# KleistLab/ADAPTed

Measured on NVIDIA B200. Metric: reads_per_sec, higher is better.
Workload: dtype f64 traces / f32 statistics / fp16-split tensor-core convolutions / i16 input

## Files before the change

adapted_b200/csrc/adb_cnn.cuh:

```cuda
#pragma once
#include "adb_series_median.cuh"
#include <cuda_fp16.h>
#include <float.h>

#include "adb_common.cuh"
#include "adb_ctx.cuh"
#include "adb_select.cuh"
#include <algorithm>

#define ADB_CNN_NPARAMS 58882
#define CNN_C 64
#define CNN_K 7
#define CNN_SCORE_EXCL (-5.0f)
#define CNN_W1 0
#define CNN_B1 (CNN_W1 + 64 * 7)
#define CNN_W2 (CNN_B1 + 64)
#define CNN_B2 (CNN_W2 + 64 * 64 * 7)
#define CNN_W3 (CNN_B2 + 64)
#define CNN_B3 (CNN_W3 + 64 * 64 * 7)
#define CNN_W4 (CNN_B3 + 64)
#define CNN_B4 (CNN_W4 + 64 * 2 * 7)

#define CNN_TILE 96
#define CNN_TILE_IN 104
#define CNN_THREADS 192

struct SmemKeys {
    const float *p;
    __device__ __forceinline__ uint32_t operator()(int j) const { return f32_key(p[j]); }
};
struct SmemDevKeys {
    const float *p;
    float med;
    __device__ __forceinline__ uint32_t operator()(int j) const { return f32_key(fabsf(__fsub_rn(p[j], med))); }
};
struct KeyF32Id {
    __device__ __forceinline__ float operator()(uint32_t k) const { return key_f32(k); }
};

template <class F>
__device__ __forceinline__ float cnn_block_mean(F f, int factor) {
    return __fdiv_rn(np_sum_f32_leaf(f, factor), (float)factor);
}

__global__ void __launch_bounds__(256) cnn_prep_kernel(BatchDev B, int A0, int f, int L, float *x) {
    extern __shared__ __align__(16) unsigned char smem[];
    float *ds = (float *)smem;
    unsigned char *scr = smem + (((size_t)L * 4 + 15) & ~(size_t)15);
    SelScratch S = sel_scratch_from(scr);
    uint32_t *kbuf = (uint32_t *)(scr + ((ADB_SEL_SMEM_BYTES + 15) & ~15));
    const int r = blockIdx.x;
    const ReadSrc src = make_src(B, r);
    int nv;
    {
        const int span = B.m - A0;
        if (span <= 0) nv = 0;
        else if (src.n >= B.m) nv = L;
        else nv = (src.n > A0) ? (src.n - A0) / f : 0;
        nv = min(nv, L);
    }
    for (int b = threadIdx.x; b < nv; b += blockDim.x) {
        const int j0 = A0 + b * f;
        ds[b] = cnn_block_mean([&](int k) { const int j = j0 + k; return (j < B.m) ? src.pa(j) : 0.0f; }, f);
    }
    __syncthreads();
    float med = CUDART_NAN_F, mad = CUDART_NAN_F;
    if (nv > 0) {
        uint32_t kmin, kmax;
        SmemKeys K{ds};
        cta_key_minmax(K, nv, kmin, kmax, S);
        med = cta_median_keys(K, KeyF32Id(), nv, kmin, kmax, S, kbuf);
        SmemDevKeys D{ds, med};
        const float dmax = fmaxf(fabsf(__fsub_rn(key_f32(kmax), med)), fabsf(__fsub_rn(key_f32(kmin), med)));
        mad = cta_median_keys(D, KeyF32Id(), nv, f32_key(0.0f), f32_key(dmax), S, kbuf);
    }
    float *xr = x + (size_t)r * L;
    for (int b = threadIdx.x; b < L; b += blockDim.x) {
        float v = CNN_SCORE_EXCL;
        if (b < nv) {
            v = __fdiv_rn(__fsub_rn(ds[b], med), mad);
            if (!(v == v)) v = CNN_SCORE_EXCL;
            else if (v == CUDART_INF_F) v = FLT_MAX;
            else if (v == -CUDART_INF_F) v = -FLT_MAX;
        }
        xr[b] = v;
    }
}

#define PREP_WARPS 4
#define PREP_CHUNK_BINS 320
__host__ __device__ inline size_t cnn_prep_warp_smem(int L) { return (size_t)PREP_WARPS * (2 * ((L + 3) & ~3) + SM_NCAND + 4) * 4; }
__global__ void __launch_bounds__(PREP_WARPS * 32) cnn_prep_warp_kernel(BatchDev B, int A0, int f, int L, float *x) {
    extern __shared__ __align__(16) unsigned char smem[];
    const int warp = threadIdx.x >> 5, lane = threadIdx.x & 31;
    const int Lp = (L + 3) & ~3;
    float *ds = (float *)smem + (size_t)warp * (2 * Lp + SM_NCAND + 4);
    uint32_t *keys = (uint32_t *)(ds + Lp), *cand = keys + Lp;
    __shared__ uint64_t pbar[PREP_WARPS];
    if (threadIdx.x < PREP_WARPS) mbar_init(&pbar[threadIdx.x], 1);
    __syncthreads();
    uint32_t pphase = 0;
    for (int r = blockIdx.x * PREP_WARPS + warp; r < B.n_reads; r += gridDim.x * PREP_WARPS) {
        const ReadSrc src = make_src(B, r);
        int nv;
        {
            const int span = B.m - A0;
            if (span <= 0) nv = 0;
            else if (src.n >= B.m) nv = L;
            else nv = (src.n > A0) ? (src.n - A0) / f : 0;
            nv = min(nv, L);
        }
        const int nvp = (nv + 3) & ~3;
        if (lane == 0) {
            const int rn = r + gridDim.x * PREP_WARPS;
            if (rn < B.n_reads) {
                const ReadSrc nx = make_src(B, rn);
                if (nx.i16 != nullptr && nx.n > A0 + 16) {
                    const uintptr_t p0 = ((uintptr_t)(nx.i16 + A0) + 15) & ~(uintptr_t)15;
                    const uint32_t nbytes = (uint32_t)(((uintptr_t)(nx.i16 + min(nx.n, B.m)) - p0) & ~(uintptr_t)15);
                    if (nbytes) asm volatile("cp.async.bulk.prefetch.L2.global [%0], %1;" ::"l"(p0), "r"(nbytes) : "memory");
                }
            }
        }
        uint32_t mn = 0xffffffffu, mx = 0u;
        {
            int16_t *raw = reinterpret_cast<int16_t *>(keys);
            const int16_t *g0 = src.i16 + A0;
            const int cbins = min(PREP_CHUNK_BINS, (Lp * 4 - 16) / (2 * f));
            const int n_have = min(src.n, B.m) - A0;
            for (int b0 = 0; b0 < nv; b0 += cbins) {
                const int nbin = min(cbins, nv - b0), ns = min(nbin * f, n_have - b0 * f);
                const int16_t *gs = g0 + (size_t)b0 * f;
                const int shift = (int)(((uintptr_t)gs & 15) >> 1);
                const int head = min((8 - shift) & 7, ns);
                const int body = (ns - head) & ~7;
                asm volatile("fence.proxy.async.shared::cta;" ::: "memory");
                __syncwarp();
                if (lane == 0 && body > 0) {
                    mbar_expect_tx(&pbar[warp], (uint32_t)body * 2);
                    tma_bulk_g2s(raw + shift + head, gs + head, (uint32_t)body * 2, &pbar[warp]);
                }
                for (int i = lane; i < head; i += 32) raw[shift + i] = gs[i];
                for (int i = head + body + lane; i < ns; i += 32) raw[shift + i] = gs[i];
                if (body > 0) { mbar_wait(&pbar[warp], pphase); pphase ^= 1; }
                __syncwarp();
                const int16_t *rs = raw + shift;
                for (int b = lane; b < nbin; b += 32) {
                    const int16_t *p = rs + b * f;
                    const int left = ns - b * f;
                    const float v = cnn_block_mean([&](int k) { return (k < left) ? __fmul_rn(__fadd_rn((float)(int)p[k], src.coff), src.cscale) : 0.0f; }, f);
                    ds[b0 + b] = v;
                    const uint32_t k0 = f32_key(v);
                    mn = min(mn, k0); mx = max(mx, k0);
                }
                __syncwarp();
            }
            for (int b = lane; b < nv; b += 32) keys[b] = f32_key(ds[b]);
        }
        if (lane < nvp - nv) keys[nv + lane] = 0xffffffffu;
        mn = __reduce_min_sync(ADB_FULL, mn);
        mx = __reduce_max_sync(ADB_FULL, mx);
        __syncwarp();
        float med = CUDART_NAN_F, mad = CUDART_NAN_F;
        if (nv > 0) {
            const SmKeys K{reinterpret_cast<const uint4 *>(keys), nullptr};
            const unsigned rank = (unsigned)(nv - 1) >> 1;
            uint32_t a, b2;
            bool hb;
            warp_select2(K, nvp >> 2, 0u, false, nvp, rank, mn, mx, cand, a, b2, hb);
            med = (nv & 1) ? key_f32(a) : __fdiv_rn(__fadd_rn(key_f32(a), key_f32(b2)), 2.0f);
            __syncwarp();
            mn = 0xffffffffu; mx = 0u;
            for (int b = lane; b < nv; b += 32) {
                const uint32_t k = f32_key(fabsf(__fsub_rn(ds[b], med)));
                keys[b] = k;
                mn = min(mn, k); mx = max(mx, k);
            }
            mn = __reduce_min_sync(ADB_FULL, mn);
            mx = __reduce_max_sync(ADB_FULL, mx);
            __syncwarp();
            warp_select2(K, nvp >> 2, 0u, false, nvp, rank, mn, mx, cand, a, b2, hb);
            mad = (nv & 1) ? key_f32(a) : __fdiv_rn(__fadd_rn(key_f32(a), key_f32(b2)), 2.0f);
        }
        float *xr = x + (size_t)r * L;
        for (int b = lane; b < L; b += 32) {
            float v = CNN_SCORE_EXCL;
            if (b < nv) {
                v = __fdiv_rn(__fsub_rn(ds[b], med), mad);
                if (!(v == v)) v = CNN_SCORE_EXCL;
                else if (v == CUDART_INF_F) v = FLT_MAX;
                else if (v == -CUDART_INF_F) v = -FLT_MAX;
            }
            xr[b] = v;
        }
        __syncwarp();
    }
}

__global__ void cnn_pack_weights_kernel(const float *w, float *packed ) {
    const int i = blockIdx.x * blockDim.x + threadIdx.x;
    if (i >= 2 * CNN_C * CNN_K * CNN_C) return;
    const int layer = i / (CNN_C * CNN_K * CNN_C);
    const int rem = i % (CNN_C * CNN_K * CNN_C);
    const int ci = rem / (CNN_K * CNN_C), k = (rem / CNN_C) % CNN_K, co = rem % CNN_C;
    const float *src = w + (layer == 0 ? CNN_W2 : CNN_W3);
    packed[i] = src[(co * CNN_C + ci) * CNN_K + k];
}

template <bool FUSE_L1>
__global__ void __launch_bounds__(CNN_THREADS, 1) cnn_conv64_kernel(const float *in, float *out, const float *packed_w,
                                                                   const float *bias, const float *w1, const float *b1,
                                                                   int n_reads, int Lx, int L1, int LP, const int *only) {
    if (only) {
        if (only[-1] == 0) return;
        const int tiles_per_read = (L1 + CNN_TILE - 1) / CNN_TILE, n_tiles = n_reads * tiles_per_read;
        bool mine = false;
        for (int tile = blockIdx.x; tile < n_tiles && !mine; tile += gridDim.x) mine = only[tile / tiles_per_read] != 0;
        if (!__syncthreads_or(mine)) return;
    }
    extern __shared__ __align__(16) float sm[];
    float *Ws = sm;
    float *Is = Ws + CNN_C * CNN_K * CNN_C;
    float *Xs = Is + CNN_C * CNN_TILE_IN;
    float *W1s = Xs + 3 * (CNN_TILE + 6) + 8;
    for (int i = threadIdx.x; i < CNN_C * CNN_K * CNN_C; i += blockDim.x) Ws[i] = packed_w[i];
    if (FUSE_L1) {
        for (int i = threadIdx.x; i < CNN_C * CNN_K; i += blockDim.x) W1s[i] = w1[i];
        for (int i = threadIdx.x; i < CNN_C; i += blockDim.x) W1s[CNN_C * CNN_K + i] = b1[i];
    }
    __syncthreads();
    const int tiles_per_read = (L1 + CNN_TILE - 1) / CNN_TILE;
    const int n_tiles = n_reads * tiles_per_read;
    const int cg = threadIdx.x / 24, tg = threadIdx.x % 24;
    const int co0 = cg * 8, tp = tg * 4;
    float bv[8];
#pragma unroll
    for (int c = 0; c < 8; c++) bv[c] = bias[co0 + c];
    for (int tile = blockIdx.x; tile < n_tiles; tile += gridDim.x) {
        const int r = tile / tiles_per_read, t0 = (tile % tiles_per_read) * CNN_TILE;
        if (only && !only[r]) continue;
        __syncthreads();
        if (FUSE_L1) {
            const float *xr = in + (size_t)r * Lx;
            const int x0 = 3 * (t0 - 3) - 3, nx = 3 * (CNN_TILE + 6) + 6;
            for (int i = threadIdx.x; i < nx; i += blockDim.x) {
                const int j = x0 + i;
                Xs[i] = (j >= 0 && j < Lx) ? xr[j] : 0.0f;
            }
            __syncthreads();
            for (int i = threadIdx.x; i < CNN_C * (CNN_TILE + 6); i += blockDim.x) {
                const int ci = i / (CNN_TILE + 6), q = i % (CNN_TILE + 6);
                const int p = t0 - 3 + q;
                float v = 0.0f;
                if (p >= 0 && p < L1) {
                    float a = W1s[CNN_C * CNN_K + ci];
#pragma unroll
                    for (int k = 0; k < CNN_K; k++) a = fmaf(W1s[ci * CNN_K + k], Xs[3 * q + k], a);
                    v = fmaxf(a, 0.0f);
                }
                Is[ci * CNN_TILE_IN + q] = v;
            }
        } else {
            const float *ar = in + (size_t)r * CNN_C * LP;
            for (int i = threadIdx.x; i < CNN_C * (CNN_TILE + 6); i += blockDim.x) {
                const int ci = i / (CNN_TILE + 6), q = i % (CNN_TILE + 6);
                const int p = t0 - 3 + q;
                Is[ci * CNN_TILE_IN + q] = (p >= 0 && p < L1) ? ar[(size_t)ci * LP + p] : 0.0f;
            }
        }
        __syncthreads();
        float acc[8][4];
#pragma unroll
        for (int c = 0; c < 8; c++)
#pragma unroll
            for (int t = 0; t < 4; t++) acc[c][t] = bv[c];
#pragma unroll 2
        for (int ci = 0; ci < CNN_C; ci++) {
            float iv[10];
            const float *ip = Is + ci * CNN_TILE_IN + tp;
#pragma unroll
            for (int q = 0; q < 10; q++) iv[q] = ip[q];
            const float *wp = Ws + ci * CNN_K * CNN_C + co0;
#pragma unroll
            for (int k = 0; k < CNN_K; k++) {
                const float4 wa = *(const float4 *)(wp + k * CNN_C);
                const float4 wb = *(const float4 *)(wp + k * CNN_C + 4);
                const float wv[8] = {wa.x, wa.y, wa.z, wa.w, wb.x, wb.y, wb.z, wb.w};
#pragma unroll
                for (int c = 0; c < 8; c++)
#pragma unroll
                    for (int t = 0; t < 4; t++) acc[c][t] = fmaf(wv[c], iv[t + k], acc[c][t]);
            }
        }
        float *orow = out + (size_t)r * CNN_C * LP;
        const int p0 = t0 + tp;
        if (p0 < L1) {
#pragma unroll
            for (int c = 0; c < 8; c++) {
                float4 v = make_float4(fmaxf(acc[c][0], 0.f), fmaxf(acc[c][1], 0.f), fmaxf(acc[c][2], 0.f), fmaxf(acc[c][3], 0.f));
                float *dst = orow + (size_t)(co0 + c) * LP + p0;
                if (p0 + 3 < LP) *(float4 *)dst = v;
                else {
                    if (p0 < LP) dst[0] = v.x;
                    if (p0 + 1 < LP) dst[1] = v.y;
                    if (p0 + 2 < LP) dst[2] = v.z;
                }
            }
        }
    }
}

__host__ __device__ inline size_t cnn_conv_smem_bytes() {
    return (size_t)(CNN_C * CNN_K * CNN_C + CNN_C * CNN_TILE_IN + 3 * (CNN_TILE + 6) + 8 + CNN_C * CNN_K + CNN_C) * 4;
}

#define CNN_CONVT_THREADS 192
__global__ void __launch_bounds__(CNN_CONVT_THREADS) cnn_convT_kernel(const float *act, const float *w4, const float *b4, int L1, int LP,
                                                        int Lout, float *scores, const int *only) {
    if (only && (only[-1] == 0 || only[blockIdx.y] == 0)) return;
    __shared__ __align__(16) float ws[CNN_C * 16];
    for (int i = threadIdx.x; i < CNN_C * 16; i += blockDim.x) {
        const int ci = i >> 4, e = i & 15, co = e >> 3, k = e & 7;
        ws[i] = (k < CNN_K) ? w4[(ci * 2 + co) * CNN_K + k] : 0.0f;
    }
    __syncthreads();
    const int r = blockIdx.y;
    const int u = blockIdx.x * blockDim.x + threadIdx.x;
    if (3 * u >= Lout) return;
    const float *ar = act + (size_t)r * CNN_C * LP;
    const float bias0 = b4[0], bias1 = b4[1];
    float o[2][3] = {{bias0, bias0, bias0}, {bias1, bias1, bias1}};
    const bool has_m = (u - 1 >= 0) && (u - 1 < L1), has_c = u < L1, has_p = u + 1 < L1;
#pragma unroll 8
    for (int ci = 0; ci < CNN_C; ci++) {
        const float *ap = ar + (size_t)ci * LP;
        const float xm = has_m ? ap[u - 1] : 0.0f, xc = has_c ? ap[u] : 0.0f, xp = has_p ? ap[u + 1] : 0.0f;
        const float4 wa = *reinterpret_cast<const float4 *>(ws + ci * 16), wb = *reinterpret_cast<const float4 *>(ws + ci * 16 + 4);
        const float4 wc = *reinterpret_cast<const float4 *>(ws + ci * 16 + 8), wd = *reinterpret_cast<const float4 *>(ws + ci * 16 + 12);
        if (has_p) { o[0][0] = fmaf(xp, wa.x, o[0][0]); o[1][0] = fmaf(xp, wc.x, o[1][0]); }
        if (has_c) { o[0][0] = fmaf(xc, wa.w, o[0][0]); o[1][0] = fmaf(xc, wc.w, o[1][0]); }
        if (has_m) { o[0][0] = fmaf(xm, wb.z, o[0][0]); o[1][0] = fmaf(xm, wd.z, o[1][0]); }
        if (has_p) { o[0][1] = fmaf(xp, wa.y, o[0][1]); o[1][1] = fmaf(xp, wc.y, o[1][1]); }
        if (has_c) { o[0][1] = fmaf(xc, wb.x, o[0][1]); o[1][1] = fmaf(xc, wd.x, o[1][1]); }
        if (has_p) { o[0][2] = fmaf(xp, wa.z, o[0][2]); o[1][2] = fmaf(xp, wc.z, o[1][2]); }
        if (has_c) { o[0][2] = fmaf(xc, wb.y, o[0][2]); o[1][2] = fmaf(xc, wd.y, o[1][2]); }
    }
#pragma unroll
    for (int c = 0; c < 3; c++) {
        const int j = 3 * u + c;
        if (j < Lout) {
            scores[((size_t)r * 2 + 0) * Lout + j] = o[0][c];
            scores[((size_t)r * 2 + 1) * Lout + j] = o[1][c];
        }
    }
}

__device__ __forceinline__ bool np_better(float v, int i, float bv, int bi) {
    const bool vn = !(v == v), bn = !(bv == bv);
    if (vn != bn) return vn;
    if (vn) return i < bi;
    return v > bv || (v == bv && i < bi);
}

__device__ int cta_argmax(const float *p, int n, float *sv, int *si) {
    float bv = -CUDART_INF_F;
    int bi = 0x7fffffff;
    for (int i = threadIdx.x; i < n; i += blockDim.x) {
        const float v = p[i];
        if (bi == 0x7fffffff || np_better(v, i, bv, bi)) { bv = v; bi = i; }
    }
#pragma unroll
    for (int o = 16; o > 0; o >>= 1) {
        const float ov = __shfl_xor_sync(ADB_FULL, bv, o);
        const int oi = __shfl_xor_sync(ADB_FULL, bi, o);
        if (oi != 0x7fffffff && (bi == 0x7fffffff || np_better(ov, oi, bv, bi))) { bv = ov; bi = oi; }
    }
    __syncthreads();
    if ((threadIdx.x & 31) == 0) { sv[threadIdx.x >> 5] = bv; si[threadIdx.x >> 5] = bi; }
    __syncthreads();
    bv = sv[0]; bi = si[0];
    for (int w = 1; w < (int)(blockDim.x >> 5); w++)
        if (si[w] != 0x7fffffff && (bi == 0x7fffffff || np_better(sv[w], si[w], bv, bi))) { bv = sv[w]; bi = si[w]; }
    __syncthreads();
    return bi == 0x7fffffff ? 0 : bi;
}

__global__ void __launch_bounds__(256) cnn_mask_kernel(float *scores, int Lout, int n_adapter_bins, int k, int *apos,
                                                       int *ppos) {
    __shared__ float sv[8];
    __shared__ int si[8];
    const int r = blockIdx.x;
    float *c0 = scores + ((size_t)r * 2) * Lout, *c1 = c0 + Lout;
    const int a = cta_argmax(c0, min(n_adapter_bins, Lout), sv, si);
    int p = 0;
    if (k >= 1) {
        for (int j = threadIdx.x; j < a; j += blockDim.x) c1[j] = CNN_SCORE_EXCL;
        __syncthreads();
        p = cta_argmax(c1, Lout, sv, si);
        if (k > 1)
            for (int j = p + 1 + threadIdx.x; j < Lout; j += blockDim.x) c1[j] = CNN_SCORE_EXCL;
    }
    if (threadIdx.x == 0) { apos[r] = a; ppos[r] = p; }
}

struct FlatView {
    const float *scores;
    int Lout;
    int r0, nr;
    __device__ __forceinline__ float at(long long g) const {
        const int rr = (int)(g / Lout), j = (int)(g % Lout);
        return scores[((size_t)(r0 + rr) * 2 + 1) * Lout + j];
    }
    __device__ __forceinline__ long long size() const { return (long long)nr * Lout; }
};

#define CNN_PK_CAP 832

__global__ void __launch_bounds__(128) cnn_peaks_kernel(const float *scores, int Lout, int batch_size, int n_reads,
                                                        long long *pk_pos, int *pk_cnt) {
    __shared__ int wcount[4];
    __shared__ int base_sh;
    const int r = blockIdx.x;
    const int mb = r / batch_size;
    FlatView V{scores, Lout, mb * batch_size, min(batch_size, n_reads - mb * batch_size)};
    const long long N = V.size();
    const long long g0 = (long long)(r - V.r0) * Lout;
    const float *rowp = scores + ((size_t)r * 2 + 1) * Lout;
    if (threadIdx.x == 0) base_sh = 0;
    __syncthreads();
    for (int jb = 0; jb < Lout; jb += blockDim.x) {
        const int j = jb + threadIdx.x;
        long long mid = -1;
        if (j < Lout) {
            const long long i = g0 + j;
            if (i >= 1 && i < N - 1) {
                auto val = [&](long long g) { const long long jj = g - g0; return (jj >= 0 && jj < Lout) ? rowp[jj] : V.at(g); };
                const float xi = rowp[j];
                if (val(i - 1) < xi) {
                    long long ia = i + 1;
                    while (ia < N - 1 && val(ia) == xi) ia++;
                    if (val(ia) < xi) mid = (i + ia - 1) / 2;
                }
            }
        }
        const unsigned m = __ballot_sync(ADB_FULL, mid >= 0);
        if ((threadIdx.x & 31) == 0) wcount[threadIdx.x >> 5] = __popc(m);
        __syncthreads();
        int off = base_sh;
        for (int w = 0; w < (int)(threadIdx.x >> 5); w++) off += wcount[w];
        if (mid >= 0) {
            const int pos = off + __popc(m & ((1u << (threadIdx.x & 31)) - 1u));
            if (pos < CNN_PK_CAP) pk_pos[(size_t)r * CNN_PK_CAP + pos] = mid;
        }
        __syncthreads();
        if (threadIdx.x == 0) base_sh += wcount[0] + wcount[1] + wcount[2] + wcount[3];
        __syncthreads();
    }
    if (threadIdx.x == 0) pk_cnt[r] = min(base_sh, CNN_PK_CAP);
}

#define CNN_WS_CAP 2560
#define CNN_WS_SORT 4096
__global__ void __launch_bounds__(128) cnn_topk_kernel(const float *scores, int Lout, int batch_size, int n_reads, int k,
                                                       int dist, const long long *pk_pos, const int *pk_cnt, int *cand,
                                                       int *ncand) {
    __shared__ long long pos[CNN_WS_CAP];
    __shared__ float hgt[CNN_WS_CAP];
    __shared__ unsigned short ord[CNN_WS_CAP];
    __shared__ unsigned char keep[CNN_WS_CAP];
    __shared__ int n_sh;
    const int r = blockIdx.x;
    const int mb = r / batch_size;
    FlatView V{scores, Lout, mb * batch_size, min(batch_size, n_reads - mb * batch_size)};
    const int rl = r - V.r0;
    __shared__ int take_sh[2];
    const int c_mid = pk_cnt[r];
    const long long lo = (long long)rl * Lout, hi = lo + Lout;
    if (threadIdx.x == 0) {
        int tl = 0, tr = 0;
        const long long *pm = pk_pos + (size_t)r * CNN_PK_CAP;
        long long first_pos = (c_mid > 0) ? pm[0] : 0x7fffffffffffffffLL, last_pos = (c_mid > 0) ? pm[c_mid - 1] : -1;
        if (rl > 0) {
            const long long *pl = pk_pos + (size_t)(r - 1) * CNN_PK_CAP;
            const int cl = pk_cnt[r - 1];
            long long nxt = first_pos;
            while (tl < cl) {
                const long long p = pl[cl - 1 - tl];
                if (!(p >= lo || (dist > 0 && nxt != 0x7fffffffffffffffLL && nxt - p < dist))) break;
                nxt = p; tl++;
                if (last_pos < 0) last_pos = p;
            }
        }
        if (rl + 1 < V.nr && dist > 0 && last_pos >= 0) {
            const long long *pr = pk_pos + (size_t)(r + 1) * CNN_PK_CAP;
            const int cr = pk_cnt[r + 1];
            long long prv = last_pos;
            while (tr < cr && pr[tr] - prv < dist) { prv = pr[tr]; tr++; }
        }
        take_sh[0] = tl; take_sh[1] = tr;
    }
    __syncthreads();
    int n = 0;
    for (int part = 0; part < 3; part++) {
        const int rr = r - 1 + part;
        int c, first;
        if (part == 0) { c = take_sh[0]; first = (c > 0) ? pk_cnt[r - 1] - c : 0; }
        else if (part == 1) { c = c_mid; first = 0; }
        else { c = take_sh[1]; first = 0; }
        for (int i = threadIdx.x; i < c; i += blockDim.x) {
            if (n + i < CNN_WS_CAP) {
                const long long p = pk_pos[(size_t)rr * CNN_PK_CAP + first + i];
                pos[n + i] = p;
                hgt[n + i] = V.at(p);
                keep[n + i] = 2;
            }
        }
        n = min(n + c, CNN_WS_CAP);
    }
    auto over = [&](int t, int i) { const float ht = hgt[t], hi_ = hgt[i]; return (ht > hi_) || (ht == hi_ && t > i); };
    __syncthreads();
    if (dist > 0) {
        bool pending = true;
        while (__syncthreads_or(pending)) {
            pending = false;
            unsigned char newst[(CNN_WS_CAP + 127) / 128];
            int cnt = 0;
            for (int i = threadIdx.x; i < n; i += blockDim.x, cnt++) {
                unsigned char st = keep[i];
                if (st == 2) {
                    bool killed = false, wait = false;
                    for (int t = i - 1; t >= 0 && pos[i] - pos[t] < dist; t--)
                        if (over(t, i)) { const unsigned char s2 = keep[t]; killed |= (s2 == 1); wait |= (s2 == 2); }
                    for (int t = i + 1; t < n && pos[t] - pos[i] < dist; t++)
                        if (over(t, i)) { const unsigned char s2 = keep[t]; killed |= (s2 == 1); wait |= (s2 == 2); }
                    if (killed) st = 0;
                    else if (!wait) st = 1;
                    else pending = true;
                }
                newst[cnt] = st;
            }
            __syncthreads();
            cnt = 0;
            for (int i = threadIdx.x; i < n; i += blockDim.x, cnt++) keep[i] = newst[cnt];
        }
    } else {
        for (int i = threadIdx.x; i < n; i += blockDim.x) keep[i] = 1;
    }
    __syncthreads();
    if (threadIdx.x == 0) n_sh = 0;
    __syncthreads();
    for (int i = threadIdx.x; i < n; i += blockDim.x)
        if (keep[i] == 1 && pos[i] >= lo && pos[i] < hi) ord[atomicAdd(&n_sh, 1)] = (unsigned short)i;
    __syncthreads();
    const int ns = n_sh;
    for (int a = threadIdx.x; a < ns; a += blockDim.x) {
        const int i = ord[a];
        const float h = hgt[i];
        int rank = 0;
        for (int b = 0; b < ns; b++) {
            const int j = ord[b];
            const float hj = hgt[j];
            rank += (hj > h) || (hj == h && j < i);
        }
        if (rank < k) cand[(size_t)r * k + rank] = (int)(pos[i] - lo);
    }
    if (threadIdx.x == 0) ncand[r] = ns;
}

__global__ void __launch_bounds__(256) cnn_shift_kernel(const int *apos, const int *ppos, const int *cand, const int *ncand,
                                                        int batch_size, int n_reads, int k, int ds, int A0, int *given) {
    __shared__ int wtot[8];
    __shared__ int carry;
    const int mb = blockIdx.x;
    const int r0 = mb * batch_size, nr = min(batch_size, n_reads - r0);
    const int stride = 1 + max(k, 1);
    if (threadIdx.x == 0) carry = 0;
    for (int i = threadIdx.x; i < nr; i += blockDim.x) {
        int *g = given + (size_t)(r0 + i) * stride;
        const int a = apos[r0 + i];
        g[0] = (a == 0) ? 0 : a * ds + A0;
        for (int t = 0; t < max(k, 1); t++) g[1 + t] = 0;
        if (k == 1) { const int p = ppos[r0 + i]; g[1] = (p == 0) ? 0 : p * ds + A0; }
    }
    __syncthreads();
    if (k <= 1) return;
    for (int base = 0; base < nr; base += blockDim.x) {
        const int i = base + threadIdx.x;
        const int has = (i < nr && ncand[r0 + i] > 0) ? 1 : 0;
        const unsigned m = __ballot_sync(ADB_FULL, has);
        if ((threadIdx.x & 31) == 0) wtot[threadIdx.x >> 5] = __popc(m);
        __syncthreads();
        int off = carry;
        for (int w = 0; w < (int)(threadIdx.x >> 5); w++) off += wtot[w];
        if (has) {
            const int row = off + __popc(m & ((1u << (threadIdx.x & 31)) - 1u));
            int *g = given + (size_t)(r0 + row) * stride;
            const int nc = min(ncand[r0 + i], k);
            for (int t = 0; t < nc; t++) {
                const int p = cand[(size_t)(r0 + i) * k + t];
                g[1 + t] = (p == 0) ? 0 : p * ds + A0;
            }
        }
        __syncthreads();
        if (threadIdx.x == 0) { int s = 0; for (int w = 0; w < 8; w++) s += wtot[w]; carry += s; }
        __syncthreads();
    }
}

struct CnnDims {
    int Lx, L1, LP, Lout;
};
static CnnDims cnn_dims(int m, int A0, int f) {
    CnnDims d;
    d.Lx = (std::max(m - A0, 0) + f - 1) / f;
    d.L1 = (d.Lx + 2 * 3 - CNN_K) / 3 + 1;
    d.LP = (d.L1 + 3) & ~3;
    d.Lout = (d.L1 - 1) * 3 - 2 * 3 + CNN_K;
    return d;
}

__global__ void cnn_tc_pack_weights_kernel(const float *w, __half *packed);
static int cnn_tc_launch_setup();
#define ADB_CT_SLOTS 4
#define ADB_CT_FLOATS (2 * 64 * 8 + 64)
__constant__ float adb_c_convT[ADB_CT_SLOTS][ADB_CT_FLOATS];

__global__ void cnn_ct_pack_kernel(const float *w4 , const float *b3, float *out) {
    const int i = blockIdx.x * blockDim.x + threadIdx.x;
    if (i < 1024) {
        const int co = i >> 9, ci = (i >> 3) & 63, k = i & 7;
        out[i] = (k < CNN_K) ? w4[(ci * 2 + co) * CNN_K + k] : 0.0f;
    } else if (i < ADB_CT_FLOATS) {
        out[i] = b3[i - 1024];
    }
}

static void cnn_tc_launch(int layer, const void *in, void *out, const __half *wp, const float *bias, const float *w1,
                          const float *b1, int n_reads, int Lx, int L1, int LP, int *redo, int sm_count, cudaStream_t st, int cslot = -1);
static size_t cnn_tc_a0t_bytes_per_read(int L1);
static int cnn_tc_a0t_rows_host(int L1);

static int cnn_forward_dev(adb_ctx *ctx, const float *x, int n, const CnnDims &D, const float *w_dev, float *scores,
                           cudaStream_t st) {
    if (ctx->cnn_w.ensure(sizeof(float) * 2 * CNN_C * CNN_K * CNN_C)) { set_err("cudaMalloc cnn weights"); return ADB_ERR_CUDA; }
    float *packed = (float *)ctx->cnn_w.p;
    {
        KernelTimer t(ctx, 6, st);
        cnn_pack_weights_kernel<<<(2 * CNN_C * CNN_K * CNN_C + 255) / 256, 256, 0, st>>>(w_dev, packed);
    }
    ctx->launches += 1;
    const size_t act_per_read = (size_t)CNN_C * D.LP * sizeof(float);
    const int chunk = (int)std::max<size_t>(1, std::min<size_t>((size_t)n, ((size_t)1 << 30) / act_per_read));
    if (ctx->cnn_act0.ensure(act_per_read * chunk) || ctx->cnn_act1.ensure(act_per_read * chunk)) {
        set_err("cudaMalloc cnn activations");
        return ADB_ERR_CUDA;
    }
    const size_t smem = cnn_conv_smem_bytes();
    CUDA_TRY(cudaFuncSetAttribute(cnn_conv64_kernel<true>, cudaFuncAttributeMaxDynamicSharedMemorySize, (int)smem));
    CUDA_TRY(cudaFuncSetAttribute(cnn_conv64_kernel<false>, cudaFuncAttributeMaxDynamicSharedMemorySize, (int)smem));
    float *a0 = (float *)ctx->cnn_act0.p, *a1 = (float *)ctx->cnn_act1.p;
    const bool use_tc = !ctx->opt_cnn_fp32;
    __half *wtc = nullptr;
    unsigned char *a0t = nullptr;
    int *redo = nullptr;
    int cslot = -1;
    if (use_tc) {
        const size_t wbytes = sizeof(__half) * 2 * CNN_K * 2 * 4096;
        if (ctx->cnn_wtc.ensure(wbytes + sizeof(int) * ((size_t)chunk + 4))) { set_err("cudaMalloc cnn tc weights"); return ADB_ERR_CUDA; }
        wtc = (__half *)ctx->cnn_wtc.p;
        redo = (int *)((unsigned char *)ctx->cnn_wtc.p + wbytes) + 4;
        {
            KernelTimer t(ctx, 6, st);
            cnn_tc_pack_weights_kernel<<<(2 * CNN_K * 4096 + 255) / 256, 256, 0, st>>>(w_dev, wtc);
        }
        ctx->launches += 1;
        if (ctx->ct_slot >= 0 && !getenv("ADB_NO_CONST_CONVT")) {
            if (ctx->cnn_ct.ensure(sizeof(float) * ADB_CT_FLOATS)) { set_err("cudaMalloc cnn constants"); return ADB_ERR_CUDA; }
            cnn_ct_pack_kernel<<<(ADB_CT_FLOATS + 255) / 256, 256, 0, st>>>(w_dev + CNN_W4, w_dev + CNN_B3, (float *)ctx->cnn_ct.p);
            CUDA_TRY(cudaMemcpyToSymbolAsync(adb_c_convT, ctx->cnn_ct.p, sizeof(float) * ADB_CT_FLOATS,
                                             sizeof(float) * ADB_CT_FLOATS * (size_t)ctx->ct_slot, cudaMemcpyDeviceToDevice, st));
            ctx->launches += 1;
            cslot = ctx->ct_slot;
        }
        if (cnn_tc_launch_setup()) { set_err("cudaFuncSetAttribute cnn tc"); return ADB_ERR_CUDA; }
        const size_t a0t_bytes = cnn_tc_a0t_bytes_per_read(D.L1) * (size_t)chunk;
        const void *before = ctx->cnn_a0t.p;
        const size_t cap_before = ctx->cnn_a0t.cap;
        if (ctx->cnn_a0t.ensure(a0t_bytes)) { set_err("cudaMalloc cnn a0t"); return ADB_ERR_CUDA; }
        if (ctx->cnn_a0t.p != before || ctx->cnn_a0t.cap != cap_before || ctx->cnn_a0t_l1 != D.L1)
            CUDA_TRY(cudaMemsetAsync(ctx->cnn_a0t.p, 0, ctx->cnn_a0t.cap, st));
        ctx->cnn_a0t_l1 = D.L1;
        a0t = (unsigned char *)ctx->cnn_a0t.p;
    }
    for (int r0 = 0; r0 < n; r0 += chunk) {
        const int nc = std::min(chunk, n - r0);
        const int tiles = nc * ((D.L1 + CNN_TILE - 1) / CNN_TILE);
        const int grid = std::max(1, std::min(tiles, ctx->sm_count));
        if (use_tc) {
            CUDA_TRY(cudaMemsetAsync(redo - 4, 0, sizeof(int) * ((size_t)nc + 4), st));
            {
                KernelTimer t(ctx, 5, st);
                cnn_tc_launch(2, x + (size_t)r0 * D.Lx, a0t, wtc, w_dev + CNN_B2, w_dev + CNN_W1, w_dev + CNN_B1, nc, D.Lx, D.L1,
                              cnn_tc_a0t_rows_host(D.L1), redo, ctx->sm_count, st);
            }
            {
                KernelTimer t(ctx, 5, st);
                cnn_tc_launch(3, a0t, scores + (size_t)r0 * 2 * D.Lout, wtc + (size_t)CNN_K * 2 * 4096, w_dev + CNN_B3,
                              w_dev + CNN_W4, w_dev + CNN_B4, nc, D.Lout, D.L1, cnn_tc_a0t_rows_host(D.L1), redo,
                              ctx->sm_count, st, cslot);
            }
            {
                KernelTimer t(ctx, 7, st);
                cnn_conv64_kernel<true><<<grid, CNN_THREADS, smem, st>>>(x + (size_t)r0 * D.Lx, a0, packed, w_dev + CNN_B2,
                                                                          w_dev + CNN_W1, w_dev + CNN_B1, nc, D.Lx, D.L1, D.LP, redo);
                cnn_conv64_kernel<false><<<grid, CNN_THREADS, smem, st>>>(a0, a1, packed + CNN_C * CNN_K * CNN_C, w_dev + CNN_B3,
                                                                           nullptr, nullptr, nc, D.Lx, D.L1, D.LP, redo);
            }
            ctx->launches += 2;
        } else {
        {
            KernelTimer t(ctx, 5, st);
            cnn_conv64_kernel<true><<<grid, CNN_THREADS, smem, st>>>(x + (size_t)r0 * D.Lx, a0, packed, w_dev + CNN_B2,
                                                                      w_dev + CNN_W1, w_dev + CNN_B1, nc, D.Lx, D.L1, D.LP, nullptr);
        }
        {
            KernelTimer t(ctx, 5, st);
            cnn_conv64_kernel<false><<<grid, CNN_THREADS, smem, st>>>(a0, a1, packed + CNN_C * CNN_K * CNN_C, w_dev + CNN_B3,
                                                                       nullptr, nullptr, nc, D.Lx, D.L1, D.LP, nullptr);
        }
        }
        {
            KernelTimer t(ctx, use_tc ? 7 : 5, st);
            dim3 g(((D.Lout + 2) / 3 + CNN_CONVT_THREADS - 1) / CNN_CONVT_THREADS, nc);
            cnn_convT_kernel<<<g, CNN_CONVT_THREADS, 0, st>>>(a1, w_dev + CNN_W4, w_dev + CNN_B4, D.L1, D.LP, D.Lout,
                                                scores + (size_t)r0 * 2 * D.Lout, use_tc ? redo : nullptr);
        }
        ctx->launches += 3;
    }
    CUDA_TRY(cudaGetLastError());
    return ADB_OK;
}

static int cnn_primary_boundaries(adb_ctx *ctx, const BatchDev &B, const adb_config &cfg, const float *w_dev, int *given,
                                  cudaStream_t st) {
    const CnnDims D = cnn_dims(B.m, cfg.min_obs_adapter, cfg.downscale_factor);
    if (D.Lx < CNN_K || D.Lout < 3 || D.Lout / 2 + 8 > CNN_PK_CAP) {
        set_err("preload window outside the range supported by the CNN kernels");
        return ADB_ERR_UNSUPPORTED;
    }
    const int n = B.n_reads, k = cfg.polya_cand_k;
    if (ctx->cnn_x.ensure(sizeof(float) * (size_t)n * D.Lx) || ctx->cnn_scores.ensure(sizeof(float) * (size_t)n * 2 * D.Lout)) {
        set_err("cudaMalloc cnn buffers");
        return ADB_ERR_CUDA;
    }
    float *x = (float *)ctx->cnn_x.p, *scores = (float *)ctx->cnn_scores.p;
    {
        const size_t smem = (((size_t)D.Lx * 4 + 15) & ~(size_t)15) + ((ADB_SEL_SMEM_BYTES + 15) & ~15) + 64;
        CUDA_TRY(cudaFuncSetAttribute(cnn_prep_kernel, cudaFuncAttributeMaxDynamicSharedMemorySize, (int)smem));
        KernelTimer t(ctx, 6, st);
        const size_t wsm = cnn_prep_warp_smem(D.Lx);
        if (B.sig_type == ADB_SIG_I16 && (int)wsm <= ctx->max_smem_optin && !getenv("ADB_PREP_CTA") &&
            (((D.Lx + 3) & ~3) * 4 - 16) / (2 * cfg.downscale_factor) >= 32) {
            CUDA_TRY(cudaFuncSetAttribute(cnn_prep_warp_kernel, cudaFuncAttributeMaxDynamicSharedMemorySize, (int)wsm));
            int occ = 0;
            CUDA_TRY(cudaOccupancyMaxActiveBlocksPerMultiprocessor(&occ, cnn_prep_warp_kernel, PREP_WARPS * 32, wsm));
            const int grid = std::max(1, std::min((n + PREP_WARPS - 1) / PREP_WARPS, ctx->sm_count * std::max(occ, 1)));
            cnn_prep_warp_kernel<<<grid, PREP_WARPS * 32, wsm, st>>>(B, cfg.min_obs_adapter, cfg.downscale_factor, D.Lx, x);
        } else {
            cnn_prep_kernel<<<n, 256, smem, st>>>(B, cfg.min_obs_adapter, cfg.downscale_factor, D.Lx, x);
        }
        ctx->launches += 1;
    }
    int rc = cnn_forward_dev(ctx, x, n, D, w_dev, scores, st);
    if (rc) return rc;
    const size_t ints = (size_t)n * (4 + std::max(k, 1));
    if (ctx->cnn_post.ensure(sizeof(long long) * (size_t)n * CNN_PK_CAP + sizeof(int) * ints + 64)) {
        set_err("cudaMalloc cnn post-processing");
        return ADB_ERR_CUDA;
    }
    long long *pk_pos = (long long *)ctx->cnn_post.p;
    int *apos = (int *)(pk_pos + (size_t)n * CNN_PK_CAP), *ppos = apos + n, *pk_cnt = ppos + n, *ncand = pk_cnt + n;
    int *cand = ncand + n;
    const int nadp = (cfg.max_obs_adapter - cfg.min_obs_adapter) / cfg.downscale_factor;
    const int n_batches = (n + B.batch_size - 1) / B.batch_size;
    {
        KernelTimer t(ctx, 6, st);
        cnn_mask_kernel<<<n, 256, 0, st>>>(scores, D.Lout, nadp, k, apos, ppos);
    }
    ctx->launches += 1;
    if (k > 1) {
        CUDA_TRY(cudaMemsetAsync(cand, 0, sizeof(int) * (size_t)n * k, st));
        {
            KernelTimer t(ctx, 6, st);
            cnn_peaks_kernel<<<n, 128, 0, st>>>(scores, D.Lout, B.batch_size, n, pk_pos, pk_cnt);
        }
        {
            KernelTimer t(ctx, 6, st);
            cnn_topk_kernel<<<n, 128, 0, st>>>(scores, D.Lout, B.batch_size, n, k, 5, pk_pos, pk_cnt, cand, ncand);
        }
        ctx->launches += 2;
    }
    {
        KernelTimer t(ctx, 6, st);
        cnn_shift_kernel<<<n_batches, 256, 0, st>>>(apos, ppos, cand, ncand, B.batch_size, n, k, cfg.downscale_factor,
                                                    cfg.min_obs_adapter, given);
    }
    ctx->launches += 1;
    CUDA_TRY(cudaGetLastError());
    return ADB_OK;
}
```

adapted_b200/csrc/adb_cnn_tc.cuh:

```cuda
#pragma once
#include <cuda_fp16.h>

#include "adb_cnn.cuh"

#define TC_WORKERS 256
#define TC_THREADS (TC_WORKERS + 64)
#define TC_THREADS2 (2 * TC_WORKERS + 64)
#define TC_ROWS 128
#define TC_RA (TC_ROWS + 8)
#define TC_NQ (TC_ROWS + 6)
#define TC_PLANE (8 * TC_RA * 16)
#define TC_WPART (8 * 64 * 16)
#define TC_WBYTES (CNN_K * 2 * TC_WPART)
#define TC_NX (3 * TC_NQ + 6)
#define TC_ITEMS (8 * TC_NQ)
#define TC_ROUNDS ((TC_ITEMS + TC_WORKERS - 1) / TC_WORKERS)
#define TC_IDESC ((1u << 4) | ((64u >> 3) << 17) | ((128u >> 4) << 24))
#define TC_IDESC2 ((1u << 4) | ((128u >> 3) << 17) | ((128u >> 4) << 24))

__global__ void cnn_tc_pack_weights_kernel(const float *w, __half *packed) {
    const int i = blockIdx.x * blockDim.x + threadIdx.x;
    if (i >= 2 * CNN_K * 4096) return;
    const int layer = i / (CNN_K * 4096), rem = i % (CNN_K * 4096);
    const int k = rem / 4096, e = rem % 4096;
    const int kc = e / 512, co = (e / 8) % 64, j = e % 8;
    const int ci = kc * 8 + j;
    const float v = (w + (layer == 0 ? CNN_W2 : CNN_W3))[(co * CNN_C + ci) * CNN_K + k];
    const __half hi = __float2half_rn(v);
    __half *dst = packed + ((size_t)(layer * CNN_K + k) * 2) * 4096 + (size_t)kc * 1024 + co * 8 + j;
    dst[0] = hi;
    dst[512] = __float2half_rn(__fsub_rn(v, __half2float(hi)));
}

__device__ __forceinline__ uint32_t tc_desc_lo(uint32_t saddr, uint32_t lbo_bytes) {
    return ((saddr >> 4) & 0x3fffu) | (((lbo_bytes >> 4) & 0x3fffu) << 16);
}
__device__ __forceinline__ uint32_t tc_desc_hi(uint32_t sbo_bytes) { return ((sbo_bytes >> 4) & 0x3fffu) | (1u << 14); }

__device__ __forceinline__ void tc_mma_f16(uint32_t d_tmem, uint32_t a_lo, uint32_t a_hi, uint32_t b_lo, uint32_t b_hi,
                                           uint32_t accumulate, uint32_t idesc = TC_IDESC) {
    asm volatile(
        "{\n\t"
        ".reg .pred p;\n\t"
        ".reg .b64 da, db;\n\t"
        "mov.b64 da, {%1, %2};\n\t"
        "mov.b64 db, {%3, %4};\n\t"
        "setp.ne.b32 p, %6, 0;\n\t"
        "tcgen05.mma.cta_group::1.kind::f16 [%0], da, db, %5, p;\n\t"
        "}\n" ::"r"(d_tmem),
        "r"(a_lo), "r"(a_hi), "r"(b_lo), "r"(b_hi), "r"(idesc), "r"(accumulate)
        : "memory");
}

__device__ __forceinline__ bool tc_elect_one() {
    uint32_t pred;
    asm volatile(
        "{\n\t"
        ".reg .pred p;\n\t"
        "elect.sync _|p, 0xffffffff;\n\t"
        "selp.u32 %0, 1, 0, p;\n\t"
        "}"
        : "=r"(pred));
    return pred != 0;
}

__device__ __forceinline__ void tc_commit(uint64_t *bar) {
    asm volatile("tcgen05.commit.cta_group::1.mbarrier::arrive::one.shared::cluster.b64 [%0];" ::"r"(smem_u32(bar)) : "memory");
}

__device__ __forceinline__ void tc_ld32(uint32_t taddr, uint32_t v[32]) {
    asm volatile(
        "tcgen05.ld.sync.aligned.32x32b.x32.b32 "
        "{%0, %1, %2, %3, %4, %5, %6, %7, %8, %9, %10, %11, %12, %13, %14, %15, "
        "%16, %17, %18, %19, %20, %21, %22, %23, %24, %25, %26, %27, %28, %29, %30, %31}, [%32];\n"
        : "=r"(v[0]), "=r"(v[1]), "=r"(v[2]), "=r"(v[3]), "=r"(v[4]), "=r"(v[5]), "=r"(v[6]), "=r"(v[7]), "=r"(v[8]),
          "=r"(v[9]), "=r"(v[10]), "=r"(v[11]), "=r"(v[12]), "=r"(v[13]), "=r"(v[14]), "=r"(v[15]), "=r"(v[16]),
          "=r"(v[17]), "=r"(v[18]), "=r"(v[19]), "=r"(v[20]), "=r"(v[21]), "=r"(v[22]), "=r"(v[23]), "=r"(v[24]),
          "=r"(v[25]), "=r"(v[26]), "=r"(v[27]), "=r"(v[28]), "=r"(v[29]), "=r"(v[30]), "=r"(v[31])
        : "r"(taddr));
    asm volatile("tcgen05.wait::ld.sync.aligned;" ::: "memory");
}

__device__ __forceinline__ bool tc_split_store(unsigned char *hi_plane, unsigned char *lo_plane, int kc, int q,
                                               const float v[8]) {
    __half2 h[4], l[4];
    bool bad = false;
#pragma unroll
    for (int j = 0; j < 4; j++) {
        const __half h0 = __float2half_rn(v[2 * j]), h1 = __float2half_rn(v[2 * j + 1]);
        const float f0 = __half2float(h0), f1 = __half2float(h1);
        bad |= !(fabsf(f0) <= 65504.0f) || !(fabsf(f1) <= 65504.0f);
        h[j] = __halves2half2(h0, h1);
        l[j] = __halves2half2(__float2half_rn(__fsub_rn(v[2 * j], f0)), __float2half_rn(__fsub_rn(v[2 * j + 1], f1)));
    }
    const size_t off = ((size_t)kc * TC_RA + q) * 16;
    *reinterpret_cast<uint4 *>(hi_plane + off) = *reinterpret_cast<const uint4 *>(h);
    *reinterpret_cast<uint4 *>(lo_plane + off) = *reinterpret_cast<const uint4 *>(l);
    return bad;
}

#define TC_A0T_PAD 4
#define TC_L3_STRIDE (TC_ROWS - 2)
__host__ __device__ inline int cnn_tc_a0t_rows(int L1) {
    const int j2 = (L1 + TC_ROWS - 1) / TC_ROWS, j3 = (L1 + TC_L3_STRIDE - 1) / TC_L3_STRIDE;
    const int w = TC_ROWS * j2 + TC_A0T_PAD, rd = TC_L3_STRIDE * (j3 - 1) + TC_NQ;
    return ((w > rd ? w : rd) + 7) & ~7;
}
#define TC_TILE_RUN (TC_NQ * 16)

__host__ __device__ inline size_t cnn_tc_smem_bytes_layer(int layer) {
    if (layer == 3)
        return (size_t)TC_WBYTES + 3 * 2 * (size_t)TC_PLANE + 1024 * 4 + 64 * 4 + 64 * 4 + 160 + 256;
    return (size_t)TC_WBYTES + 2 * 2 * (size_t)TC_PLANE + (size_t)(TC_NX + 10) * 4 + 64 * 8 * 4 + 64 * 4 + 160 + 1024;
}

template <int LAYER, int CSLOT = -1>
__global__ void __launch_bounds__(LAYER == 2 ? TC_THREADS2 : TC_THREADS, 1) cnn_conv64_tc_kernel(const void *in, void *out, const __half *wp,
                                                                     const float *bias, const float *w1, const float *b1,
                                                                     int n_reads, int Lx, int L1, int LP, int *redo) {
    constexpr int NBUF = LAYER == 3 ? 3 : 2;
    constexpr int NWW = LAYER == 2 ? 2 * TC_WORKERS / 32 : TC_WORKERS / 32;
    const int a0t_rows = LP;
    const size_t a0t_read_bytes = (size_t)2 * 8 * a0t_rows * 16;
    extern __shared__ __align__(1024) unsigned char tsm[];
    unsigned char *Wsm = tsm;
    unsigned char *Abuf = tsm + TC_WBYTES;
    float *Xs = (float *)(Abuf + NBUF * 2 * TC_PLANE);
    float *W1s = Xs + TC_NX + 10;
    float *W4s = Xs;
    float *Eg = W4s + 1024;
    float *Bs = (LAYER == 3 ? Eg + 64 : W1s + 64 * 8);
    uint64_t *accb = (uint64_t *)(((uintptr_t)(Bs + 64) + 15) & ~(uintptr_t)15);
    uint64_t *afull = accb + 2, *accfree = accb + 2 + NBUF;
    uint64_t *sfree = accfree + 2;
    uint32_t *tmem_slot = (uint32_t *)(sfree + NBUF);
    const int tid = threadIdx.x, warp = tid >> 5, lane = tid & 31;

    if (tid == 0) {
        for (int b = 0; b < 2; b++) { mbar_init(&accb[b], 1); mbar_init(&accfree[b], TC_WORKERS); }
        for (int b = 0; b < NBUF; b++) { mbar_init(&afull[b], LAYER == 3 ? 1 : TC_WORKERS); mbar_init(&sfree[b], 1); }
    }
    for (int i = tid; i < TC_WBYTES / 16; i += blockDim.x)
        reinterpret_cast<uint4 *>(Wsm)[i] = reinterpret_cast<const uint4 *>(wp)[i];
    if (LAYER == 2) {
        for (int i = tid; i < CNN_C * CNN_K; i += blockDim.x) W1s[i] = w1[i];
        for (int i = tid; i < CNN_C; i += blockDim.x) W1s[CNN_C * CNN_K + i] = b1[i];
    } else {
        for (int i = tid; i < 1024; i += blockDim.x) {
            const int co = i >> 9, ci = (i >> 3) & 63, k = i & 7;
            W4s[i] = (k < CNN_K) ? w1[(ci * 2 + co) * CNN_K + k] : 0.0f;
        }
    }
    if (tid < CNN_C) Bs[tid] = bias[tid];
    if (warp == 0) {
        asm volatile("tcgen05.alloc.cta_group::1.sync.aligned.shared::cta.b32 [%0], %1;" ::"r"(smem_u32(tmem_slot)), "r"(256));
        asm volatile("tcgen05.relinquish_alloc_permit.cta_group::1.sync.aligned;");
    }
    asm volatile("fence.proxy.async.shared::cta;" ::: "memory");
    asm volatile("tcgen05.fence::before_thread_sync;" ::: "memory");
    __syncthreads();
    asm volatile("tcgen05.fence::after_thread_sync;" ::: "memory");
    const uint32_t tmem = *tmem_slot;

    const int jobs_per_read = LAYER == 3 ? (L1 + TC_L3_STRIDE - 1) / TC_L3_STRIDE : (L1 + TC_ROWS - 1) / TC_ROWS;
    const int n_jobs = n_reads * jobs_per_read;

    float px[2];
    float w1r[8][CNN_K], b1r[8];
    if (LAYER == 2 && warp < TC_WORKERS / 32) {
#pragma unroll
        for (int j = 0; j < 8; j++) {
            b1r[j] = W1s[CNN_C * CNN_K + warp * 8 + j];
#pragma unroll
            for (int k = 0; k < CNN_K; k++) w1r[j][k] = W1s[(warp * 8 + j) * CNN_K + k];
        }
    }
    auto prefetch = [&](int job) {
        const int r = job / jobs_per_read, t0 = (job % jobs_per_read) * TC_ROWS;
        const float *xr = (const float *)in + (size_t)r * Lx;
        const int x0 = 3 * (t0 - 3) - 3;
#pragma unroll
        for (int u = 0; u < 2; u++) {
            const int i = tid + u * TC_WORKERS, j = x0 + i;
            px[u] = (i < TC_NX && j >= 0 && j < Lx) ? xr[j] : 0.0f;
        }
    };
    auto build = [&](int job, int b) {
        const int r = job / jobs_per_read, t0 = (job % jobs_per_read) * TC_ROWS;
        unsigned char *hi_plane = Abuf + (size_t)b * 2 * TC_PLANE, *lo_plane = hi_plane + TC_PLANE;
        bool bad = false;
        asm volatile("bar.sync 1, %0;" ::"n"(TC_WORKERS) : "memory");
#pragma unroll
        for (int u = 0; u < 2; u++) {
            const int i = tid + u * TC_WORKERS;
            if (i < TC_NX) Xs[i] = px[u];
        }
        asm volatile("bar.sync 1, %0;" ::"n"(TC_WORKERS) : "memory");
        for (int q = lane; q < TC_NQ; q += 32) {
            const int p = t0 - 3 + q;
            float v[8] = {0.f, 0.f, 0.f, 0.f, 0.f, 0.f, 0.f, 0.f};
            if (p >= 0 && p < L1) {
                float xs[CNN_K];
#pragma unroll
                for (int k = 0; k < CNN_K; k++) xs[k] = Xs[3 * q + k];
#pragma unroll
                for (int j = 0; j < 8; j++) {
                    float a = b1r[j];
#pragma unroll
                    for (int k = 0; k < CNN_K; k++) a = fmaf(w1r[j][k], xs[k], a);
                    v[j] = fmaxf(a, 0.0f);
                }
            }
            bad |= tc_split_store(hi_plane, lo_plane, warp, q, v);
        }
        if (bad) { redo[r] = 1; redo[-1] = 1; }
        asm volatile("fence.proxy.async.shared::cta;" ::: "memory");
        asm volatile("mbarrier.arrive.shared::cta.b64 _, [%0];" ::"r"(smem_u32(&afull[b])) : "memory");
    };
    auto load_tile = [&](int job, int b) {
        const int r = job / jobs_per_read, rho0 = (job % jobs_per_read) * TC_L3_STRIDE;
        const unsigned char *src = (const unsigned char *)in + (size_t)r * a0t_read_bytes + (size_t)rho0 * 16;
        unsigned char *dst = Abuf + (size_t)b * 2 * TC_PLANE;
        mbar_expect_tx(&afull[b], 16 * TC_TILE_RUN);
#pragma unroll 1
        for (int pk = 0; pk < 16; pk++)
            tma_bulk_g2s(dst + (size_t)pk * (TC_RA * 16), src + (size_t)pk * ((size_t)a0t_rows * 16), TC_TILE_RUN, &afull[b]);
    };
    const uint32_t w_lo0 = tc_desc_lo(smem_u32(Wsm), 128 * 16), w_hi = tc_desc_hi(128);
    const uint32_t a_hi_word = tc_desc_hi(128);
    auto issue = [&](int sb, int tb) {
        const uint32_t ah0 = tc_desc_lo(smem_u32(Abuf + (size_t)sb * 2 * TC_PLANE), TC_RA * 16);
        const uint32_t al0 = ah0 + (TC_PLANE >> 4);
        const uint32_t d = tmem + (uint32_t)(tb * 128);
#pragma unroll
        for (int k = 0; k < CNN_K; k++) {
#pragma unroll
            for (int kp = 0; kp < 4; kp++) {
                const uint32_t a_off = (uint32_t)((2 * kp) * TC_RA + k);
                const uint32_t w_off = (uint32_t)(((k * 2) * TC_WPART + 2 * kp * 128 * 16) >> 4);
                tc_mma_f16(d, ah0 + a_off, a_hi_word, w_lo0 + w_off, w_hi, (k > 0 || kp > 0) ? 1u : 0u, TC_IDESC2);
                tc_mma_f16(d, al0 + a_off, a_hi_word, w_lo0 + w_off, w_hi, 1u, TC_IDESC);
            }
        }
        tc_commit(&accb[tb]);
    };
    auto epilogue = [&](int job, int tb, uint32_t phase, int eb) {
        const int r = job / jobs_per_read;
        const int t0 = LAYER == 3 ? (job % jobs_per_read) * TC_L3_STRIDE - 1 : (job % jobs_per_read) * TC_ROWS;
        mbar_wait(&accb[tb], phase);
        asm volatile("tcgen05.fence::after_thread_sync;" ::: "memory");
        const int q = (warp & 3) * 32 + lane, ch0 = ((warp >> 2) & 1) * 32;
        const int p = t0 + q;
        uint32_t v[32];
        if (LAYER == 3) {
            const int co = warp >> 2, wq = warp & 3;
            const uint32_t taddr = tmem + ((uint32_t)(wq * 32) << 16) + (uint32_t)(tb * 128);
            const bool live = p >= 0 && p < L1;
            float P[CNN_K] = {0.f, 0.f, 0.f, 0.f, 0.f, 0.f, 0.f};
            const float4 *wv = reinterpret_cast<const float4 *>(W4s + co * 512);
#pragma unroll
            for (int hh = 0; hh < 2; hh++) {
                tc_ld32(taddr + (uint32_t)(hh * 32), v);
                {
                    uint32_t v2[32];
                    tc_ld32(taddr + (uint32_t)(64 + hh * 32), v2);
#pragma unroll
                    for (int c = 0; c < 32; c++) v[c] = __float_as_uint(__fadd_rn(__uint_as_float(v[c]), __uint_as_float(v2[c])));
                }
                if (hh == 1) {
                    asm volatile("tcgen05.fence::before_thread_sync;" ::: "memory");
                    asm volatile("mbarrier.arrive.shared::cta.b64 _, [%0];" ::"r"(smem_u32(&accfree[tb])) : "memory");
                }
                if (CSLOT >= 0) {
                    auto acc = [&](const float *cw, const float *cb) {
#pragma unroll
                        for (int c = 0; c < 32; c++) {
                            const int ci = hh * 32 + c;
                            const float a = live ? fmaxf(__fadd_rn(__uint_as_float(v[c]), cb[ci]), 0.0f) : 0.0f;
#pragma unroll
                            for (int j = 0; j < CNN_K; j++) P[j] = fmaf(a, cw[ci * 8 + j], P[j]);
                        }
                    };
                    constexpr int SL = CSLOT >= 0 ? CSLOT : 0;
                    if (co == 0) acc(&adb_c_convT[SL][0], &adb_c_convT[SL][1024]);
                    else acc(&adb_c_convT[SL][512], &adb_c_convT[SL][1024]);
                } else {
#pragma unroll
                    for (int c = 0; c < 32; c++) {
                        const int ci = hh * 32 + c;
                        const float a = live ? fmaxf(__fadd_rn(__uint_as_float(v[c]), Bs[ci]), 0.0f) : 0.0f;
                        const float4 w0 = wv[ci * 2], w1v = wv[ci * 2 + 1];
                        P[0] = fmaf(a, w0.x, P[0]); P[1] = fmaf(a, w0.y, P[1]); P[2] = fmaf(a, w0.z, P[2]); P[3] = fmaf(a, w0.w, P[3]);
                        P[4] = fmaf(a, w1v.x, P[4]); P[5] = fmaf(a, w1v.y, P[5]); P[6] = fmaf(a, w1v.z, P[6]);
                    }
                }
            }
            float up0 = __shfl_down_sync(ADB_FULL, P[0], 1), up1 = __shfl_down_sync(ADB_FULL, P[1], 1);
            float up2 = __shfl_down_sync(ADB_FULL, P[2], 1), dn6 = __shfl_up_sync(ADB_FULL, P[6], 1);
            float *eg = Eg + ((eb * 2 + co) * 4) * 4;
            if (lane == 0) { eg[wq * 4 + 0] = P[0]; eg[wq * 4 + 1] = P[1]; eg[wq * 4 + 2] = P[2]; }
            if (lane == 31) eg[wq * 4 + 3] = P[6];
            asm volatile("bar.sync 1, %0;" ::"n"(TC_WORKERS) : "memory");
            if (lane == 31 && wq < 3) { up0 = eg[(wq + 1) * 4 + 0]; up1 = eg[(wq + 1) * 4 + 1]; up2 = eg[(wq + 1) * 4 + 2]; }
            if (lane == 0 && wq > 0) dn6 = eg[(wq - 1) * 4 + 3];
            const int Lout = Lx;
            if (q >= 1 && q <= TC_L3_STRIDE && p < L1 && 3 * p < Lout) {
                const float bco = b1[co];
                float *orow = (float *)out + ((size_t)r * 2 + co) * Lout + 3 * p;
                orow[0] = __fadd_rn(bco, __fadd_rn(__fadd_rn(up0, P[3]), dn6));
                if (3 * p + 1 < Lout) orow[1] = __fadd_rn(bco, __fadd_rn(up1, P[4]));
                if (3 * p + 2 < Lout) orow[2] = __fadd_rn(bco, __fadd_rn(up2, P[5]));
            }
        } else {
            const uint32_t taddr = tmem + ((uint32_t)((warp & 3) * 32) << 16) + (uint32_t)(tb * 128 + ch0);
            tc_ld32(taddr, v);
            {
                uint32_t v2[32];
                tc_ld32(taddr + 64u, v2);
#pragma unroll
                for (int c = 0; c < 32; c++) v[c] = __float_as_uint(__fadd_rn(__uint_as_float(v[c]), __uint_as_float(v2[c])));
            }
            unsigned char *base = (unsigned char *)out + (size_t)r * a0t_read_bytes + (size_t)(p + TC_A0T_PAD) * 16;
            bool bad = false;
#pragma unroll
            for (int o = 0; o < 4; o++) {
                __half2 h[4], l[4];
#pragma unroll
                for (int j = 0; j < 4; j++) {
                    float f0 = fmaxf(__fadd_rn(__uint_as_float(v[8 * o + 2 * j]), Bs[ch0 + 8 * o + 2 * j]), 0.0f);
                    float f1 = fmaxf(__fadd_rn(__uint_as_float(v[8 * o + 2 * j + 1]), Bs[ch0 + 8 * o + 2 * j + 1]), 0.0f);
                    if (p >= L1) { f0 = 0.0f; f1 = 0.0f; }
                    const __half h0 = __float2half_rn(f0), h1 = __float2half_rn(f1);
                    const float g0 = __half2float(h0), g1 = __half2float(h1);
                    bad |= !(fabsf(g0) <= 65504.0f) || !(fabsf(g1) <= 65504.0f);
                    h[j] = __halves2half2(h0, h1);
                    l[j] = __halves2half2(__float2half_rn(__fsub_rn(f0, g0)), __float2half_rn(__fsub_rn(f1, g1)));
                }
                const size_t off = (size_t)((ch0 >> 3) + o) * ((size_t)a0t_rows * 16);
                *reinterpret_cast<uint4 *>(base + off) = *reinterpret_cast<const uint4 *>(h);
                *reinterpret_cast<uint4 *>(base + (size_t)8 * ((size_t)a0t_rows * 16) + off) = *reinterpret_cast<const uint4 *>(l);
            }
            if (bad) { redo[r] = 1; redo[-1] = 1; }
        }
    };

    if (warp == NWW) {
        if (tc_elect_one()) {
            uint32_t it = 0;
            for (int job = blockIdx.x; job < n_jobs; job += gridDim.x, it++) {
                const int tb = (int)(it & 1u), sb = (int)(it % NBUF);
                mbar_wait(&afull[sb], (it / NBUF) & 1u);
                if (it >= 2) mbar_wait(&accfree[tb], ((it - 2) >> 1) & 1u);
                asm volatile("tcgen05.fence::after_thread_sync;" ::: "memory");
                issue(sb, tb);
                if (LAYER == 3) tc_commit(&sfree[sb]);
            }
        }
        __syncwarp();
    } else if (warp == NWW + 1) {
        if (LAYER == 3 && lane == 0) {
            uint32_t it = 0;
            for (int job = blockIdx.x; job < n_jobs; job += gridDim.x, it++) {
                const int sb = (int)(it % NBUF);
                if (it >= NBUF) mbar_wait(&sfree[sb], ((it / NBUF) - 1) & 1u);
                load_tile(job, sb);
            }
        }
        __syncwarp();
    } else {
        if (LAYER == 2) {
            if (warp < TC_WORKERS / 32) {
                int job = blockIdx.x;
                if (job < n_jobs) {
                    prefetch(job);
                    build(job, 0);
                    if (job + (int)gridDim.x < n_jobs) prefetch(job + (int)gridDim.x);
                }
                uint32_t it = 0;
                for (; job < n_jobs; job += gridDim.x, it++) {
                    const int b = (int)(it & 1u);
                    const int next = job + (int)gridDim.x;
                    if (next < n_jobs) {
                        if (it >= 1) mbar_wait(&accb[b ^ 1], ((it - 1) >> 1) & 1u);
                        build(next, b ^ 1);
                        if (next + (int)gridDim.x < n_jobs) prefetch(next + (int)gridDim.x);
                    }
                }
            } else {
                uint32_t it = 0;
                for (int job = blockIdx.x; job < n_jobs; job += gridDim.x, it++) {
                    const int tb = (int)(it & 1u);
                    epilogue(job, tb, (it >> 1) & 1u, tb);
                    asm volatile("tcgen05.fence::before_thread_sync;" ::: "memory");
                    asm volatile("mbarrier.arrive.shared::cta.b64 _, [%0];" ::"r"(smem_u32(&accfree[tb])) : "memory");
                }
            }
        } else {
            int prev_job = -1;
            uint32_t it = 0;
            for (int job = blockIdx.x; job < n_jobs; job += gridDim.x, it++) {
                const int b = (int)(it & 1u);
                if (prev_job >= 0) epilogue(prev_job, b ^ 1, ((it - 1) >> 1) & 1u, b ^ 1);
                prev_job = job;
            }
            if (prev_job >= 0) epilogue(prev_job, (int)((it - 1) & 1u), ((it - 1) >> 1) & 1u, (int)((it - 1) & 1u));
        }
    }
    asm volatile("tcgen05.fence::before_thread_sync;" ::: "memory");
    __syncthreads();
    if (warp == 0) asm volatile("tcgen05.dealloc.cta_group::1.sync.aligned.b32 %0, %1;" ::"r"(tmem), "r"(256));
}

static int cnn_tc_launch_setup() {
    if (cudaFuncSetAttribute(cnn_conv64_tc_kernel<2>, cudaFuncAttributeMaxDynamicSharedMemorySize, (int)cnn_tc_smem_bytes_layer(2)) != cudaSuccess) return -1;
    if (cudaFuncSetAttribute(cnn_conv64_tc_kernel<3>, cudaFuncAttributeMaxDynamicSharedMemorySize, (int)cnn_tc_smem_bytes_layer(3)) != cudaSuccess) return -1;
    if (cudaFuncSetAttribute(cnn_conv64_tc_kernel<3, 0>, cudaFuncAttributeMaxDynamicSharedMemorySize, (int)cnn_tc_smem_bytes_layer(3)) != cudaSuccess) return -1;
    if (cudaFuncSetAttribute(cnn_conv64_tc_kernel<3, 1>, cudaFuncAttributeMaxDynamicSharedMemorySize, (int)cnn_tc_smem_bytes_layer(3)) != cudaSuccess) return -1;
    if (cudaFuncSetAttribute(cnn_conv64_tc_kernel<3, 2>, cudaFuncAttributeMaxDynamicSharedMemorySize, (int)cnn_tc_smem_bytes_layer(3)) != cudaSuccess) return -1;
    if (cudaFuncSetAttribute(cnn_conv64_tc_kernel<3, 3>, cudaFuncAttributeMaxDynamicSharedMemorySize, (int)cnn_tc_smem_bytes_layer(3)) != cudaSuccess) return -1;
    return 0;
}

static void cnn_tc_launch(int layer, const void *in, void *out, const __half *wp, const float *bias, const float *w1,
                          const float *b1, int n_reads, int Lx, int L1, int LP, int *redo, int sm_count, cudaStream_t st,
                          int cslot) {
    const int jobs = n_reads * (layer == 3 ? (L1 + TC_L3_STRIDE - 1) / TC_L3_STRIDE : (L1 + TC_ROWS - 1) / TC_ROWS);
    const int grid = std::max(1, std::min(jobs, sm_count));
    const size_t smem = cnn_tc_smem_bytes_layer(layer);
    if (layer == 2) cnn_conv64_tc_kernel<2><<<grid, TC_THREADS2, smem, st>>>(in, out, wp, bias, w1, b1, n_reads, Lx, L1, LP, redo);
    else if (cslot == 0) cnn_conv64_tc_kernel<3, 0><<<grid, TC_THREADS, smem, st>>>(in, out, wp, bias, w1, b1, n_reads, Lx, L1, LP, redo);
    else if (cslot == 1) cnn_conv64_tc_kernel<3, 1><<<grid, TC_THREADS, smem, st>>>(in, out, wp, bias, w1, b1, n_reads, Lx, L1, LP, redo);
    else if (cslot == 2) cnn_conv64_tc_kernel<3, 2><<<grid, TC_THREADS, smem, st>>>(in, out, wp, bias, w1, b1, n_reads, Lx, L1, LP, redo);
    else if (cslot == 3) cnn_conv64_tc_kernel<3, 3><<<grid, TC_THREADS, smem, st>>>(in, out, wp, bias, w1, b1, n_reads, Lx, L1, LP, redo);
    else cnn_conv64_tc_kernel<3><<<grid, TC_THREADS, smem, st>>>(in, out, wp, bias, w1, b1, n_reads, Lx, L1, LP, redo);
}

static size_t cnn_tc_a0t_bytes_per_read(int L1) { return (size_t)2 * 8 * cnn_tc_a0t_rows(L1) * 16; }
static int cnn_tc_a0t_rows_host(int L1) { return cnn_tc_a0t_rows(L1); }
```

adapted_b200/csrc/build.py:

```python
from __future__ import annotations

import os
import subprocess
import sys

HERE = os.path.dirname(os.path.abspath(__file__))
SO = os.path.join(HERE, "libadapted_b200.so")
SOURCES = ["adb_api.cu", "adb_csv.cpp"]
FLAGS = [
    "-gencode", "arch=compute_100a,code=sm_100a", "-O3", "-lineinfo", "-std=c++17",
    "-fmad=false",
    "-Xcompiler", "-fPIC", "-shared", "-Xptxas", "-v",
]


def needs_build() -> bool:
    if not os.path.exists(SO):
        return True
    t = os.path.getmtime(SO)
    deps = [os.path.join(HERE, f) for f in os.listdir(HERE) if f.endswith((".cu", ".cuh", ".cpp"))]
    deps.append(os.path.join(HERE, "..", "..", "include", "adapted_b200.h"))
    return any(os.path.getmtime(d) > t for d in deps)


def build(force: bool = False, verbose: bool = False) -> str:
    if not force and not needs_build():
        return SO
    nvcc = os.environ.get("NVCC", "/usr/local/cuda/bin/nvcc")
    cmd = [nvcc, *FLAGS, *[os.path.join(HERE, s) for s in SOURCES], "-o", SO]
    res = subprocess.run(cmd, capture_output=True, text=True)
    if verbose or res.returncode != 0:
        sys.stderr.write(res.stdout + res.stderr)
    if res.returncode != 0:
        raise RuntimeError("nvcc failed building libadapted_b200.so")
    with open(os.path.join(HERE, "ptxas_info.txt"), "w") as f:
        f.write(res.stderr)
    return SO


if __name__ == "__main__":
    print(build(force=True, verbose="-v" in sys.argv))
```

Measured before the change: 2.360 million.

## Quadruple-buffer TMEM accumulators and widen layer-3 epilogue in CNN tensor-core kernel

Layer 3 of the tensor-core conv kernel now runs with four TMEM accumulator buffers and twice the epilogue warps. Each epilogue group handles both output channels for alternating jobs. Layer 2's drainer frees its accumulator right after the TMEM loads, which it now issues as paired loads, and the builder double-buffers its input window to drop one barrier. The transposed-conv kernel uses a grid-stride loop over reads capped at twice the SM count. Optional clock-based phase instrumentation and a build option for defines are added. The risks are more TMEM and thread usage per CTA and more complex barrier phase logic.

```diff
diff --git a/adapted_b200/csrc/adb_cnn.cuh b/adapted_b200/csrc/adb_cnn.cuh
--- a/adapted_b200/csrc/adb_cnn.cuh
+++ b/adapted_b200/csrc/adb_cnn.cuh
@@ -315,42 +315,44 @@
 }
 
 #define CNN_CONVT_THREADS 192
-__global__ void __launch_bounds__(CNN_CONVT_THREADS) cnn_convT_kernel(const float *act, const float *w4, const float *b4, int L1, int LP,
-                                                        int Lout, float *scores, const int *only) {
-    if (only && (only[-1] == 0 || only[blockIdx.y] == 0)) return;
+__global__ void __launch_bounds__(CNN_CONVT_THREADS) cnn_convT_kernel(const float *act, const float *w4, const float *b4, int n_reads,
+                                                        int L1, int LP, int Lout, float *scores, const int *only) {
+    if (only && only[-1] == 0) return;
     __shared__ __align__(16) float ws[CNN_C * 16];
     for (int i = threadIdx.x; i < CNN_C * 16; i += blockDim.x) {
         const int ci = i >> 4, e = i & 15, co = e >> 3, k = e & 7;
         ws[i] = (k < CNN_K) ? w4[(ci * 2 + co) * CNN_K + k] : 0.0f;
     }
     __syncthreads();
-    const int r = blockIdx.y;
     const int u = blockIdx.x * blockDim.x + threadIdx.x;
     if (3 * u >= Lout) return;
-    const float *ar = act + (size_t)r * CNN_C * LP;
-    const float bias0 = b4[0], bias1 = b4[1];
-    float o[2][3] = {{bias0, bias0, bias0}, {bias1, bias1, bias1}};
-    const bool has_m = (u - 1 >= 0) && (u - 1 < L1), has_c = u < L1, has_p = u + 1 < L1;
+    for (int r = blockIdx.y; r < n_reads; r += gridDim.y) {
+        if (only && only[r] == 0) continue;
+        const float *ar = act + (size_t)r * CNN_C * LP;
+        const float bias0 = b4[0], bias1 = b4[1];
+        float o[2][3] = {{bias0, bias0, bias0}, {bias1, bias1, bias1}};
+        const bool has_m = (u - 1 >= 0) && (u - 1 < L1), has_c = u < L1, has_p = u + 1 < L1;
 #pragma unroll 8
-    for (int ci = 0; ci < CNN_C; ci++) {
-        const float *ap = ar + (size_t)ci * LP;
-        const float xm = has_m ? ap[u - 1] : 0.0f, xc = has_c ? ap[u] : 0.0f, xp = has_p ? ap[u + 1] : 0.0f;
-        const float4 wa = *reinterpret_cast<const float4 *>(ws + ci * 16), wb = *reinterpret_cast<const float4 *>(ws + ci * 16 + 4);
-        const float4 wc = *reinterpret_cast<const float4 *>(ws + ci * 16 + 8), wd = *reinterpret_cast<const float4 *>(ws + ci * 16 + 12);
-        if (has_p) { o[0][0] = fmaf(xp, wa.x, o[0][0]); o[1][0] = fmaf(xp, wc.x, o[1][0]); }
-        if (has_c) { o[0][0] = fmaf(xc, wa.w, o[0][0]); o[1][0] = fmaf(xc, wc.w, o[1][0]); }
-        if (has_m) { o[0][0] = fmaf(xm, wb.z, o[0][0]); o[1][0] = fmaf(xm, wd.z, o[1][0]); }
-        if (has_p) { o[0][1] = fmaf(xp, wa.y, o[0][1]); o[1][1] = fmaf(xp, wc.y, o[1][1]); }
-        if (has_c) { o[0][1] = fmaf(xc, wb.x, o[0][1]); o[1][1] = fmaf(xc, wd.x, o[1][1]); }
-        if (has_p) { o[0][2] = fmaf(xp, wa.z, o[0][2]); o[1][2] = fmaf(xp, wc.z, o[1][2]); }
-        if (has_c) { o[0][2] = fmaf(xc, wb.y, o[0][2]); o[1][2] = fmaf(xc, wd.y, o[1][2]); }
-    }
-#pragma unroll
-    for (int c = 0; c < 3; c++) {
-        const int j = 3 * u + c;
-        if (j < Lout) {
-            scores[((size_t)r * 2 + 0) * Lout + j] = o[0][c];
-            scores[((size_t)r * 2 + 1) * Lout + j] = o[1][c];
+        for (int ci = 0; ci < CNN_C; ci++) {
+            const float *ap = ar + (size_t)ci * LP;
+            const float xm = has_m ? ap[u - 1] : 0.0f, xc = has_c ? ap[u] : 0.0f, xp = has_p ? ap[u + 1] : 0.0f;
+            const float4 wa = *reinterpret_cast<const float4 *>(ws + ci * 16), wb = *reinterpret_cast<const float4 *>(ws + ci * 16 + 4);
+            const float4 wc = *reinterpret_cast<const float4 *>(ws + ci * 16 + 8), wd = *reinterpret_cast<const float4 *>(ws + ci * 16 + 12);
+            if (has_p) { o[0][0] = fmaf(xp, wa.x, o[0][0]); o[1][0] = fmaf(xp, wc.x, o[1][0]); }
+            if (has_c) { o[0][0] = fmaf(xc, wa.w, o[0][0]); o[1][0] = fmaf(xc, wc.w, o[1][0]); }
+            if (has_m) { o[0][0] = fmaf(xm, wb.z, o[0][0]); o[1][0] = fmaf(xm, wd.z, o[1][0]); }
+            if (has_p) { o[0][1] = fmaf(xp, wa.y, o[0][1]); o[1][1] = fmaf(xp, wc.y, o[1][1]); }
+            if (has_c) { o[0][1] = fmaf(xc, wb.x, o[0][1]); o[1][1] = fmaf(xc, wd.x, o[1][1]); }
+            if (has_p) { o[0][2] = fmaf(xp, wa.z, o[0][2]); o[1][2] = fmaf(xp, wc.z, o[1][2]); }
+            if (has_c) { o[0][2] = fmaf(xc, wb.y, o[0][2]); o[1][2] = fmaf(xc, wd.y, o[1][2]); }
+        }
+#pragma unroll
+        for (int c = 0; c < 3; c++) {
+            const int j = 3 * u + c;
+            if (j < Lout) {
+                scores[((size_t)r * 2 + 0) * Lout + j] = o[0][c];
+                scores[((size_t)r * 2 + 1) * Lout + j] = o[1][c];
+            }
         }
     }
 }
@@ -731,8 +733,8 @@
         }
         {
             KernelTimer t(ctx, use_tc ? 7 : 5, st);
-            dim3 g(((D.Lout + 2) / 3 + CNN_CONVT_THREADS - 1) / CNN_CONVT_THREADS, nc);
-            cnn_convT_kernel<<<g, CNN_CONVT_THREADS, 0, st>>>(a1, w_dev + CNN_W4, w_dev + CNN_B4, D.L1, D.LP, D.Lout,
+            dim3 g(((D.Lout + 2) / 3 + CNN_CONVT_THREADS - 1) / CNN_CONVT_THREADS, use_tc ? std::min(nc, 2 * ctx->sm_count) : nc);
+            cnn_convT_kernel<<<g, CNN_CONVT_THREADS, 0, st>>>(a1, w_dev + CNN_W4, w_dev + CNN_B4, nc, D.L1, D.LP, D.Lout,
                                                 scores + (size_t)r0 * 2 * D.Lout, use_tc ? redo : nullptr);
         }
         ctx->launches += 3;
diff --git a/adapted_b200/csrc/adb_cnn_tc.cuh b/adapted_b200/csrc/adb_cnn_tc.cuh
--- a/adapted_b200/csrc/adb_cnn_tc.cuh
+++ b/adapted_b200/csrc/adb_cnn_tc.cuh
@@ -4,8 +4,7 @@
 #include "adb_cnn.cuh"
 
 #define TC_WORKERS 256
-#define TC_THREADS (TC_WORKERS + 64)
-#define TC_THREADS2 (2 * TC_WORKERS + 64)
+#define TC_THREADS (2 * TC_WORKERS + 64)
 #define TC_ROWS 128
 #define TC_RA (TC_ROWS + 8)
 #define TC_NQ (TC_ROWS + 6)
@@ -68,18 +67,61 @@
     asm volatile("tcgen05.commit.cta_group::1.mbarrier::arrive::one.shared::cluster.b64 [%0];" ::"r"(smem_u32(bar)) : "memory");
 }
 
-__device__ __forceinline__ void tc_ld32(uint32_t taddr, uint32_t v[32]) {
+__device__ __forceinline__ void tc_ld32x2(uint32_t taddr_a, uint32_t taddr_b, uint32_t a[32], uint32_t b[32]) {
     asm volatile(
         "tcgen05.ld.sync.aligned.32x32b.x32.b32 "
         "{%0, %1, %2, %3, %4, %5, %6, %7, %8, %9, %10, %11, %12, %13, %14, %15, "
-        "%16, %17, %18, %19, %20, %21, %22, %23, %24, %25, %26, %27, %28, %29, %30, %31}, [%32];\n"
-        : "=r"(v[0]), "=r"(v[1]), "=r"(v[2]), "=r"(v[3]), "=r"(v[4]), "=r"(v[5]), "=r"(v[6]), "=r"(v[7]), "=r"(v[8]),
-          "=r"(v[9]), "=r"(v[10]), "=r"(v[11]), "=r"(v[12]), "=r"(v[13]), "=r"(v[14]), "=r"(v[15]), "=r"(v[16]),
-          "=r"(v[17]), "=r"(v[18]), "=r"(v[19]), "=r"(v[20]), "=r"(v[21]), "=r"(v[22]), "=r"(v[23]), "=r"(v[24]),
-          "=r"(v[25]), "=r"(v[26]), "=r"(v[27]), "=r"(v[28]), "=r"(v[29]), "=r"(v[30]), "=r"(v[31])
-        : "r"(taddr));
-    asm volatile("tcgen05.wait::ld.sync.aligned;" ::: "memory");
-}
+        "%16, %17, %18, %19, %20, %21, %22, %23, %24, %25, %26, %27, %28, %29, %30, %31}, [%64];\n\t"
+        "tcgen05.ld.sync.aligned.32x32b.x32.b32 "
+        "{%32, %33, %34, %35, %36, %37, %38, %39, %40, %41, %42, %43, %44, %45, %46, %47, "
+        "%48, %49, %50, %51, %52, %53, %54, %55, %56, %57, %58, %59, %60, %61, %62, %63}, [%65];\n\t"
+        "tcgen05.wait::ld.sync.aligned;\n"
+        : "=r"(a[0]), "=r"(a[1]), "=r"(a[2]), "=r"(a[3]), "=r"(a[4]), "=r"(a[5]), "=r"(a[6]), "=r"(a[7]), "=r"(a[8]),
+          "=r"(a[9]), "=r"(a[10]), "=r"(a[11]), "=r"(a[12]), "=r"(a[13]), "=r"(a[14]), "=r"(a[15]), "=r"(a[16]),
+          "=r"(a[17]), "=r"(a[18]), "=r"(a[19]), "=r"(a[20]), "=r"(a[21]), "=r"(a[22]), "=r"(a[23]), "=r"(a[24]),
+          "=r"(a[25]), "=r"(a[26]), "=r"(a[27]), "=r"(a[28]), "=r"(a[29]), "=r"(a[30]), "=r"(a[31]),
+          "=r"(b[0]), "=r"(b[1]), "=r"(b[2]), "=r"(b[3]), "=r"(b[4]), "=r"(b[5]), "=r"(b[6]), "=r"(b[7]), "=r"(b[8]),
+          "=r"(b[9]), "=r"(b[10]), "=r"(b[11]), "=r"(b[12]), "=r"(b[13]), "=r"(b[14]), "=r"(b[15]), "=r"(b[16]),
+          "=r"(b[17]), "=r"(b[18]), "=r"(b[19]), "=r"(b[20]), "=r"(b[21]), "=r"(b[22]), "=r"(b[23]), "=r"(b[24]),
+          "=r"(b[25]), "=r"(b[26]), "=r"(b[27]), "=r"(b[28]), "=r"(b[29]), "=r"(b[30]), "=r"(b[31])
+        : "r"(taddr_a), "r"(taddr_b)
+        : "memory");
+}
+
+__device__ __forceinline__ void tc_ld16x2(uint32_t taddr_a, uint32_t taddr_b, uint32_t a[16], uint32_t b[16]) {
+    asm volatile(
+        "tcgen05.ld.sync.aligned.32x32b.x16.b32 "
+        "{%0, %1, %2, %3, %4, %5, %6, %7, %8, %9, %10, %11, %12, %13, %14, %15}, [%32];\n\t"
+        "tcgen05.ld.sync.aligned.32x32b.x16.b32 "
+        "{%16, %17, %18, %19, %20, %21, %22, %23, %24, %25, %26, %27, %28, %29, %30, %31}, [%33];\n\t"
+        "tcgen05.wait::ld.sync.aligned;\n"
+        : "=r"(a[0]), "=r"(a[1]), "=r"(a[2]), "=r"(a[3]), "=r"(a[4]), "=r"(a[5]), "=r"(a[6]), "=r"(a[7]), "=r"(a[8]),
+          "=r"(a[9]), "=r"(a[10]), "=r"(a[11]), "=r"(a[12]), "=r"(a[13]), "=r"(a[14]), "=r"(a[15]),
+          "=r"(b[0]), "=r"(b[1]), "=r"(b[2]), "=r"(b[3]), "=r"(b[4]), "=r"(b[5]), "=r"(b[6]), "=r"(b[7]), "=r"(b[8]),
+          "=r"(b[9]), "=r"(b[10]), "=r"(b[11]), "=r"(b[12]), "=r"(b[13]), "=r"(b[14]), "=r"(b[15])
+        : "r"(taddr_a), "r"(taddr_b)
+        : "memory");
+}
+
+struct TcPhases {
+#ifdef ADB_CNN_PHASE_CLOCKS
+    long long sum[4] = {0, 0, 0, 0}, t = 0;
+    int tiles = 0;
+    __device__ __forceinline__ void start() { t = clock64(); }
+    __device__ __forceinline__ void lap(int i) { const long long c = clock64(); sum[i] += c - t; t = c; }
+    __device__ __forceinline__ void tile() { tiles++; }
+    __device__ void report(int layer, const char *role, const char *p0, const char *p1, const char *p2, const char *p3) const {
+        if (blockIdx.x == 0)
+            printf("ADB_PHASE layer=%d role=%s warp=%d tiles=%d %s=%lld %s=%lld %s=%lld %s=%lld\n", layer, role,
+                   (int)(threadIdx.x >> 5), tiles, p0, sum[0], p1, sum[1], p2, sum[2], p3, sum[3]);
+    }
+#else
+    __device__ __forceinline__ void start() {}
+    __device__ __forceinline__ void lap(int) {}
+    __device__ __forceinline__ void tile() {}
+    __device__ __forceinline__ void report(int, const char *, const char *, const char *, const char *, const char *) const {}
+#endif
+};
 
 __device__ __forceinline__ bool tc_split_store(unsigned char *hi_plane, unsigned char *lo_plane, int kc, int q,
                                                const float v[8]) {
@@ -108,36 +150,40 @@
 }
 #define TC_TILE_RUN (TC_NQ * 16)
 
-__host__ __device__ inline size_t cnn_tc_smem_bytes_layer(int layer) {
-    if (layer == 3)
-        return (size_t)TC_WBYTES + 3 * 2 * (size_t)TC_PLANE + 1024 * 4 + 64 * 4 + 64 * 4 + 160 + 256;
-    return (size_t)TC_WBYTES + 2 * 2 * (size_t)TC_PLANE + (size_t)(TC_NX + 10) * 4 + 64 * 8 * 4 + 64 * 4 + 160 + 1024;
-}
+#define TC_EG_FLOATS 256
+__host__ __device__ constexpr size_t cnn_tc_smem_bytes_layer(int layer) {
+    return layer == 3
+               ? (size_t)TC_WBYTES + 3 * 2 * (size_t)TC_PLANE + 1024 * 4 + TC_EG_FLOATS * 4 + 64 * 4 + 160 + 256
+               : (size_t)TC_WBYTES + 2 * 2 * (size_t)TC_PLANE + 2 * (size_t)(TC_NX + 10) * 4 + 64 * 8 * 4 + 64 * 4 + 160 + 1024;
+}
+static_assert(cnn_tc_smem_bytes_layer(2) <= 232448 && cnn_tc_smem_bytes_layer(3) <= 232448, "cnn_conv64_tc_kernel shared memory");
+static_assert(cnn_tc_smem_bytes_layer(3) + 1024 > 233472 / 2, "a layer-3 CTA must be alone on its SM");
 
 template <int LAYER, int CSLOT = -1>
-__global__ void __launch_bounds__(LAYER == 2 ? TC_THREADS2 : TC_THREADS, 1) cnn_conv64_tc_kernel(const void *in, void *out, const __half *wp,
+__global__ void __launch_bounds__(TC_THREADS, 1) cnn_conv64_tc_kernel(const void *in, void *out, const __half *wp,
                                                                      const float *bias, const float *w1, const float *b1,
                                                                      int n_reads, int Lx, int L1, int LP, int *redo) {
     constexpr int NBUF = LAYER == 3 ? 3 : 2;
-    constexpr int NWW = LAYER == 2 ? 2 * TC_WORKERS / 32 : TC_WORKERS / 32;
+    constexpr int NACC = LAYER == 3 ? 4 : 2;
+    constexpr int NWW = 2 * TC_WORKERS / 32;
     const int a0t_rows = LP;
     const size_t a0t_read_bytes = (size_t)2 * 8 * a0t_rows * 16;
     extern __shared__ __align__(1024) unsigned char tsm[];
     unsigned char *Wsm = tsm;
     unsigned char *Abuf = tsm + TC_WBYTES;
     float *Xs = (float *)(Abuf + NBUF * 2 * TC_PLANE);
-    float *W1s = Xs + TC_NX + 10;
+    float *W1s = Xs + 2 * (TC_NX + 10);
     float *W4s = Xs;
     float *Eg = W4s + 1024;
-    float *Bs = (LAYER == 3 ? Eg + 64 : W1s + 64 * 8);
+    float *Bs = (LAYER == 3 ? Eg + TC_EG_FLOATS : W1s + 64 * 8);
     uint64_t *accb = (uint64_t *)(((uintptr_t)(Bs + 64) + 15) & ~(uintptr_t)15);
-    uint64_t *afull = accb + 2, *accfree = accb + 2 + NBUF;
-    uint64_t *sfree = accfree + 2;
+    uint64_t *afull = accb + NACC, *accfree = accb + NACC + NBUF;
+    uint64_t *sfree = accfree + NACC;
     uint32_t *tmem_slot = (uint32_t *)(sfree + NBUF);
     const int tid = threadIdx.x, warp = tid >> 5, lane = tid & 31;
 
     if (tid == 0) {
-        for (int b = 0; b < 2; b++) { mbar_init(&accb[b], 1); mbar_init(&accfree[b], TC_WORKERS); }
+        for (int b = 0; b < NACC; b++) { mbar_init(&accb[b], 1); mbar_init(&accfree[b], LAYER == 3 ? 128 : TC_WORKERS); }
         for (int b = 0; b < NBUF; b++) { mbar_init(&afull[b], LAYER == 3 ? 1 : TC_WORKERS); mbar_init(&sfree[b], 1); }
     }
     for (int i = tid; i < TC_WBYTES / 16; i += blockDim.x)
@@ -153,7 +199,7 @@
     }
     if (tid < CNN_C) Bs[tid] = bias[tid];
     if (warp == 0) {
-        asm volatile("tcgen05.alloc.cta_group::1.sync.aligned.shared::cta.b32 [%0], %1;" ::"r"(smem_u32(tmem_slot)), "r"(256));
+        asm volatile("tcgen05.alloc.cta_group::1.sync.aligned.shared::cta.b32 [%0], %1;" ::"r"(smem_u32(tmem_slot)), "r"(NACC * 128));
         asm volatile("tcgen05.relinquish_alloc_permit.cta_group::1.sync.aligned;");
     }
     asm volatile("fence.proxy.async.shared::cta;" ::: "memory");
@@ -161,6 +207,7 @@
     __syncthreads();
     asm volatile("tcgen05.fence::after_thread_sync;" ::: "memory");
     const uint32_t tmem = *tmem_slot;
+    TcPhases ph;
 
     const int jobs_per_read = LAYER == 3 ? (L1 + TC_L3_STRIDE - 1) / TC_L3_STRIDE : (L1 + TC_ROWS - 1) / TC_ROWS;
     const int n_jobs = n_reads * jobs_per_read;
@@ -185,24 +232,30 @@
             px[u] = (i < TC_NX && j >= 0 && j < Lx) ? xr[j] : 0.0f;
         }
     };
+    int xw_parity = 0;
     auto build = [&](int job, int b) {
         const int r = job / jobs_per_read, t0 = (job % jobs_per_read) * TC_ROWS;
         unsigned char *hi_plane = Abuf + (size_t)b * 2 * TC_PLANE, *lo_plane = hi_plane + TC_PLANE;
+        float *xw = Xs + xw_parity * (TC_NX + 10);
+        xw_parity ^= 1;
         bool bad = false;
-        asm volatile("bar.sync 1, %0;" ::"n"(TC_WORKERS) : "memory");
+        ph.start();
 #pragma unroll
         for (int u = 0; u < 2; u++) {
             const int i = tid + u * TC_WORKERS;
-            if (i < TC_NX) Xs[i] = px[u];
+            if (i < TC_NX) xw[i] = px[u];
         }
         asm volatile("bar.sync 1, %0;" ::"n"(TC_WORKERS) : "memory");
-        for (int q = lane; q < TC_NQ; q += 32) {
+        ph.lap(1);
+#pragma unroll
+        for (int q = lane; q < 32 * ((TC_NQ + 31) / 32); q += 32) {
+            if (q >= TC_NQ) break;
             const int p = t0 - 3 + q;
             float v[8] = {0.f, 0.f, 0.f, 0.f, 0.f, 0.f, 0.f, 0.f};
             if (p >= 0 && p < L1) {
                 float xs[CNN_K];
 #pragma unroll
-                for (int k = 0; k < CNN_K; k++) xs[k] = Xs[3 * q + k];
+                for (int k = 0; k < CNN_K; k++) xs[k] = xw[3 * q + k];
 #pragma unroll
                 for (int j = 0; j < 8; j++) {
                     float a = b1r[j];
@@ -216,6 +269,7 @@
         if (bad) { redo[r] = 1; redo[-1] = 1; }
         asm volatile("fence.proxy.async.shared::cta;" ::: "memory");
         asm volatile("mbarrier.arrive.shared::cta.b64 _, [%0];" ::"r"(smem_u32(&afull[b])) : "memory");
+        ph.lap(2);
     };
     auto load_tile = [&](int job, int b) {
         const int r = job / jobs_per_read, rho0 = (job % jobs_per_read) * TC_L3_STRIDE;
@@ -247,79 +301,104 @@
     auto epilogue = [&](int job, int tb, uint32_t phase, int eb) {
         const int r = job / jobs_per_read;
         const int t0 = LAYER == 3 ? (job % jobs_per_read) * TC_L3_STRIDE - 1 : (job % jobs_per_read) * TC_ROWS;
+        ph.start();
         mbar_wait(&accb[tb], phase);
         asm volatile("tcgen05.fence::after_thread_sync;" ::: "memory");
+        ph.lap(0);
         const int q = (warp & 3) * 32 + lane, ch0 = ((warp >> 2) & 1) * 32;
         const int p = t0 + q;
         uint32_t v[32];
         if (LAYER == 3) {
-            const int co = warp >> 2, wq = warp & 3;
+            const int wq = warp & 3, g = warp >> 2;
             const uint32_t taddr = tmem + ((uint32_t)(wq * 32) << 16) + (uint32_t)(tb * 128);
             const bool live = p >= 0 && p < L1;
-            float P[CNN_K] = {0.f, 0.f, 0.f, 0.f, 0.f, 0.f, 0.f};
-            const float4 *wv = reinterpret_cast<const float4 *>(W4s + co * 512);
-#pragma unroll
-            for (int hh = 0; hh < 2; hh++) {
-                tc_ld32(taddr + (uint32_t)(hh * 32), v);
+            float P[2][CNN_K] = {{0.f, 0.f, 0.f, 0.f, 0.f, 0.f, 0.f}, {0.f, 0.f, 0.f, 0.f, 0.f, 0.f, 0.f}};
+            constexpr int NH = CSLOT >= 0 ? 2 : 4, HW = 64 / NH;
+#pragma unroll(CSLOT >= 0 ? NH : 1)
+            for (int hh = 0; hh < NH; hh++) {
                 {
-                    uint32_t v2[32];
-                    tc_ld32(taddr + (uint32_t)(64 + hh * 32), v2);
-#pragma unroll
-                    for (int c = 0; c < 32; c++) v[c] = __float_as_uint(__fadd_rn(__uint_as_float(v[c]), __uint_as_float(v2[c])));
-                }
-                if (hh == 1) {
+                    uint32_t v2[HW];
+                    if constexpr (HW == 32) tc_ld32x2(taddr + (uint32_t)(hh * HW), taddr + (uint32_t)(64 + hh * HW), v, v2);
+                    else tc_ld16x2(taddr + (uint32_t)(hh * HW), taddr + (uint32_t)(64 + hh * HW), v, v2);
+#pragma unroll
+                    for (int c = 0; c < HW; c++) v[c] = __float_as_uint(__fadd_rn(__uint_as_float(v[c]), __uint_as_float(v2[c])));
+                }
+                if (hh == NH - 1) {
                     asm volatile("tcgen05.fence::before_thread_sync;" ::: "memory");
                     asm volatile("mbarrier.arrive.shared::cta.b64 _, [%0];" ::"r"(smem_u32(&accfree[tb])) : "memory");
                 }
+                ph.lap(1);
                 if (CSLOT >= 0) {
-                    auto acc = [&](const float *cw, const float *cb) {
-#pragma unroll
-                        for (int c = 0; c < 32; c++) {
-                            const int ci = hh * 32 + c;
-                            const float a = live ? fmaxf(__fadd_rn(__uint_as_float(v[c]), cb[ci]), 0.0f) : 0.0f;
-#pragma unroll
-                            for (int j = 0; j < CNN_K; j++) P[j] = fmaf(a, cw[ci * 8 + j], P[j]);
+                    constexpr int SL = CSLOT >= 0 ? CSLOT : 0;
+                    const float *cw = &adb_c_convT[SL][0], *cb = &adb_c_convT[SL][1024];
+#pragma unroll
+                    for (int c = 0; c < HW; c++) {
+                        const int ci = hh * HW + c;
+                        const float a = live ? fmaxf(__fadd_rn(__uint_as_float(v[c]), cb[ci]), 0.0f) : 0.0f;
+#pragma unroll
+                        for (int co = 0; co < 2; co++)
+#pragma unroll
+                            for (int j = 0; j < CNN_K; j++) P[co][j] = fmaf(a, cw[co * 512 + ci * 8 + j], P[co][j]);
+                    }
+                } else {
+#pragma unroll
+                    for (int c = 0; c < HW; c++) {
+                        const int ci = hh * HW + c;
+                        const float a = live ? fmaxf(__fadd_rn(__uint_as_float(v[c]), Bs[ci]), 0.0f) : 0.0f;
+#pragma unroll
+                        for (int co = 0; co < 2; co++) {
+                            const float4 *wv = reinterpret_cast<const float4 *>(W4s + co * 512 + ci * 8);
+                            const float4 w0 = wv[0], w1v = wv[1];
+                            P[co][0] = fmaf(a, w0.x, P[co][0]); P[co][1] = fmaf(a, w0.y, P[co][1]);
+                            P[co][2] = fmaf(a, w0.z, P[co][2]); P[co][3] = fmaf(a, w0.w, P[co][3]);
+                            P[co][4] = fmaf(a, w1v.x, P[co][4]); P[co][5] = fmaf(a, w1v.y, P[co][5]);
+                            P[co][6] = fmaf(a, w1v.z, P[co][6]);
                         }
-                    };
-                    constexpr int SL = CSLOT >= 0 ? CSLOT : 0;
-                    if (co == 0) acc(&adb_c_convT[SL][0], &adb_c_convT[SL][1024]);
-                    else acc(&adb_c_convT[SL][512], &adb_c_convT[SL][1024]);
-                } else {
-#pragma unroll
-                    for (int c = 0; c < 32; c++) {
-                        const int ci = hh * 32 + c;
-                        const float a = live ? fmaxf(__fadd_rn(__uint_as_float(v[c]), Bs[ci]), 0.0f) : 0.0f;
-                        const float4 w0 = wv[ci * 2], w1v = wv[ci * 2 + 1];
-                        P[0] = fmaf(a, w0.x, P[0]); P[1] = fmaf(a, w0.y, P[1]); P[2] = fmaf(a, w0.z, P[2]); P[3] = fmaf(a, w0.w, P[3]);
-                        P[4] = fmaf(a, w1v.x, P[4]); P[5] = fmaf(a, w1v.y, P[5]); P[6] = fmaf(a, w1v.z, P[6]);
                     }
                 }
-            }
-            float up0 = __shfl_down_sync(ADB_FULL, P[0], 1), up1 = __shfl_down_sync(ADB_FULL, P[1], 1);
-            float up2 = __shfl_down_sync(ADB_FULL, P[2], 1), dn6 = __shfl_up_sync(ADB_FULL, P[6], 1);
-            float *eg = Eg + ((eb * 2 + co) * 4) * 4;
-            if (lane == 0) { eg[wq * 4 + 0] = P[0]; eg[wq * 4 + 1] = P[1]; eg[wq * 4 + 2] = P[2]; }
-            if (lane == 31) eg[wq * 4 + 3] = P[6];
-            asm volatile("bar.sync 1, %0;" ::"n"(TC_WORKERS) : "memory");
-            if (lane == 31 && wq < 3) { up0 = eg[(wq + 1) * 4 + 0]; up1 = eg[(wq + 1) * 4 + 1]; up2 = eg[(wq + 1) * 4 + 2]; }
-            if (lane == 0 && wq > 0) dn6 = eg[(wq - 1) * 4 + 3];
+                ph.lap(2);
+            }
+            float up[2][3], dn6[2];
+            float *eg = Eg + ((g * 2 + eb) * 2) * 16;
+#pragma unroll
+            for (int co = 0; co < 2; co++) {
+#pragma unroll
+                for (int j = 0; j < 3; j++) up[co][j] = __shfl_down_sync(ADB_FULL, P[co][j], 1);
+                dn6[co] = __shfl_up_sync(ADB_FULL, P[co][6], 1);
+                float *e = eg + co * 16 + wq * 4;
+                if (lane == 0) { e[0] = P[co][0]; e[1] = P[co][1]; e[2] = P[co][2]; }
+                if (lane == 31) e[3] = P[co][6];
+            }
+            asm volatile("bar.sync %0, 128;" ::"r"(1 + g) : "memory");
+#pragma unroll
+            for (int co = 0; co < 2; co++) {
+                const float *e = eg + co * 16;
+                if (lane == 31 && wq < 3) { up[co][0] = e[(wq + 1) * 4 + 0]; up[co][1] = e[(wq + 1) * 4 + 1]; up[co][2] = e[(wq + 1) * 4 + 2]; }
+                if (lane == 0 && wq > 0) dn6[co] = e[(wq - 1) * 4 + 3];
+            }
             const int Lout = Lx;
             if (q >= 1 && q <= TC_L3_STRIDE && p < L1 && 3 * p < Lout) {
-                const float bco = b1[co];
-                float *orow = (float *)out + ((size_t)r * 2 + co) * Lout + 3 * p;
-                orow[0] = __fadd_rn(bco, __fadd_rn(__fadd_rn(up0, P[3]), dn6));
-                if (3 * p + 1 < Lout) orow[1] = __fadd_rn(bco, __fadd_rn(up1, P[4]));
-                if (3 * p + 2 < Lout) orow[2] = __fadd_rn(bco, __fadd_rn(up2, P[5]));
-            }
+#pragma unroll
+                for (int co = 0; co < 2; co++) {
+                    const float bco = b1[co];
+                    float *orow = (float *)out + ((size_t)r * 2 + co) * Lout + 3 * p;
+                    orow[0] = __fadd_rn(bco, __fadd_rn(__fadd_rn(up[co][0], P[co][3]), dn6[co]));
+                    if (3 * p + 1 < Lout) orow[1] = __fadd_rn(bco, __fadd_rn(up[co][1], P[co][4]));
+                    if (3 * p + 2 < Lout) orow[2] = __fadd_rn(bco, __fadd_rn(up[co][2], P[co][5]));
+                }
+            }
+            ph.lap(3);
         } else {
             const uint32_t taddr = tmem + ((uint32_t)((warp & 3) * 32) << 16) + (uint32_t)(tb * 128 + ch0);
-            tc_ld32(taddr, v);
             {
                 uint32_t v2[32];
-                tc_ld32(taddr + 64u, v2);
+                tc_ld32x2(taddr, taddr + 64u, v, v2);
 #pragma unroll
                 for (int c = 0; c < 32; c++) v[c] = __float_as_uint(__fadd_rn(__uint_as_float(v[c]), __uint_as_float(v2[c])));
             }
+            asm volatile("tcgen05.fence::before_thread_sync;" ::: "memory");
+            asm volatile("mbarrier.arrive.shared::cta.b64 _, [%0];" ::"r"(smem_u32(&accfree[tb])) : "memory");
+            ph.lap(1);
             unsigned char *base = (unsigned char *)out + (size_t)r * a0t_read_bytes + (size_t)(p + TC_A0T_PAD) * 16;
             bool bad = false;
 #pragma unroll
@@ -341,6 +420,7 @@
                 *reinterpret_cast<uint4 *>(base + (size_t)8 * ((size_t)a0t_rows * 16) + off) = *reinterpret_cast<const uint4 *>(l);
             }
             if (bad) { redo[r] = 1; redo[-1] = 1; }
+            ph.lap(3);
         }
     };
 
@@ -348,13 +428,19 @@
         if (tc_elect_one()) {
             uint32_t it = 0;
             for (int job = blockIdx.x; job < n_jobs; job += gridDim.x, it++) {
-                const int tb = (int)(it & 1u), sb = (int)(it % NBUF);
+                const int tb = (int)(it % NACC), sb = (int)(it % NBUF);
+                ph.start();
                 mbar_wait(&afull[sb], (it / NBUF) & 1u);
-                if (it >= 2) mbar_wait(&accfree[tb], ((it - 2) >> 1) & 1u);
+                ph.lap(0);
+                if (it >= NACC) mbar_wait(&accfree[tb], ((it - NACC) / NACC) & 1u);
+                ph.lap(1);
                 asm volatile("tcgen05.fence::after_thread_sync;" ::: "memory");
                 issue(sb, tb);
                 if (LAYER == 3) tc_commit(&sfree[sb]);
-            }
+                ph.lap(2);
+                ph.tile();
+            }
+            ph.report(LAYER, "issuer", "wait_afull", "wait_accfree", "issue", "-");
         }
         __syncwarp();
     } else if (warp == NWW + 1) {
@@ -381,34 +467,38 @@
                     const int b = (int)(it & 1u);
                     const int next = job + (int)gridDim.x;
                     if (next < n_jobs) {
+                        ph.start();
                         if (it >= 1) mbar_wait(&accb[b ^ 1], ((it - 1) >> 1) & 1u);
+                        ph.lap(0);
                         build(next, b ^ 1);
                         if (next + (int)gridDim.x < n_jobs) prefetch(next + (int)gridDim.x);
+                        ph.lap(3);
+                        ph.tile();
                     }
                 }
+                if (lane == 0) ph.report(LAYER, "builder", "wait_accb", "x_window", "layer1_split_store", "prefetch");
             } else {
                 uint32_t it = 0;
                 for (int job = blockIdx.x; job < n_jobs; job += gridDim.x, it++) {
-                    const int tb = (int)(it & 1u);
-                    epilogue(job, tb, (it >> 1) & 1u, tb);
-                    asm volatile("tcgen05.fence::before_thread_sync;" ::: "memory");
-                    asm volatile("mbarrier.arrive.shared::cta.b64 _, [%0];" ::"r"(smem_u32(&accfree[tb])) : "memory");
-                }
+                    const int tb = (int)(it % NACC);
+                    epilogue(job, tb, (it / NACC) & 1u, tb);
+                    ph.tile();
+                }
+                if (lane == 0) ph.report(LAYER, "drainer", "wait_accb", "tmem_ld", "-", "relu_split_store");
             }
         } else {
-            int prev_job = -1;
-            uint32_t it = 0;
-            for (int job = blockIdx.x; job < n_jobs; job += gridDim.x, it++) {
-                const int b = (int)(it & 1u);
-                if (prev_job >= 0) epilogue(prev_job, b ^ 1, ((it - 1) >> 1) & 1u, b ^ 1);
-                prev_job = job;
-            }
-            if (prev_job >= 0) epilogue(prev_job, (int)((it - 1) & 1u), ((it - 1) >> 1) & 1u, (int)((it - 1) & 1u));
+            const int g = warp >> 2;
+            uint32_t it = (uint32_t)g;
+            for (int job = blockIdx.x + g * (int)gridDim.x; job < n_jobs; job += NACC * (int)gridDim.x, it += NACC) {
+                epilogue(job, g, (it / NACC) & 1u, (int)((it / NACC) & 1u));
+                ph.tile();
+            }
+            if (lane == 0) ph.report(LAYER, "epilogue", "wait_accb", "tmem_ld", "arith", "shfl_barrier_store");
         }
     }
     asm volatile("tcgen05.fence::before_thread_sync;" ::: "memory");
     __syncthreads();
-    if (warp == 0) asm volatile("tcgen05.dealloc.cta_group::1.sync.aligned.b32 %0, %1;" ::"r"(tmem), "r"(256));
+    if (warp == 0) asm volatile("tcgen05.dealloc.cta_group::1.sync.aligned.b32 %0, %1;" ::"r"(tmem), "r"(NACC * 128));
 }
 
 static int cnn_tc_launch_setup() {
@@ -427,7 +517,7 @@
     const int jobs = n_reads * (layer == 3 ? (L1 + TC_L3_STRIDE - 1) / TC_L3_STRIDE : (L1 + TC_ROWS - 1) / TC_ROWS);
     const int grid = std::max(1, std::min(jobs, sm_count));
     const size_t smem = cnn_tc_smem_bytes_layer(layer);
-    if (layer == 2) cnn_conv64_tc_kernel<2><<<grid, TC_THREADS2, smem, st>>>(in, out, wp, bias, w1, b1, n_reads, Lx, L1, LP, redo);
+    if (layer == 2) cnn_conv64_tc_kernel<2><<<grid, TC_THREADS, smem, st>>>(in, out, wp, bias, w1, b1, n_reads, Lx, L1, LP, redo);
     else if (cslot == 0) cnn_conv64_tc_kernel<3, 0><<<grid, TC_THREADS, smem, st>>>(in, out, wp, bias, w1, b1, n_reads, Lx, L1, LP, redo);
     else if (cslot == 1) cnn_conv64_tc_kernel<3, 1><<<grid, TC_THREADS, smem, st>>>(in, out, wp, bias, w1, b1, n_reads, Lx, L1, LP, redo);
     else if (cslot == 2) cnn_conv64_tc_kernel<3, 2><<<grid, TC_THREADS, smem, st>>>(in, out, wp, bias, w1, b1, n_reads, Lx, L1, LP, redo);
diff --git a/adapted_b200/csrc/build.py b/adapted_b200/csrc/build.py
--- a/adapted_b200/csrc/build.py
+++ b/adapted_b200/csrc/build.py
@@ -23,19 +23,19 @@
     return any(os.path.getmtime(d) > t for d in deps)
 
 
-def build(force: bool = False, verbose: bool = False) -> str:
-    if not force and not needs_build():
+def build(force: bool = False, verbose: bool = False, out: str = SO, defines: tuple = ()) -> str:
+    if out == SO and not force and not needs_build():
         return SO
     nvcc = os.environ.get("NVCC", "/usr/local/cuda/bin/nvcc")
-    cmd = [nvcc, *FLAGS, *[os.path.join(HERE, s) for s in SOURCES], "-o", SO]
+    cmd = [nvcc, *FLAGS, *["-D" + d for d in defines], *[os.path.join(HERE, s) for s in SOURCES], "-o", out]
     res = subprocess.run(cmd, capture_output=True, text=True)
     if verbose or res.returncode != 0:
         sys.stderr.write(res.stdout + res.stderr)
     if res.returncode != 0:
         raise RuntimeError("nvcc failed building libadapted_b200.so")
-    with open(os.path.join(HERE, "ptxas_info.txt"), "w") as f:
+    with open(os.path.join(os.path.dirname(os.path.abspath(out)), "ptxas_info.txt"), "w") as f:
         f.write(res.stderr)
-    return SO
+    return out
 
 
 if __name__ == "__main__":
```

Result: faster. 2.398 million, median of 6 (+1.6%).
